# danieleschmidt/AV-Separation-Transformer

Hardware: NVIDIA B200
Metric: separated utterance-sec/sec (higher is better)
Workload: dtype bf16

## Files before the change

av-separation-transformer_b200/csrc/avsep_api.cu:

```cuda
#include "../../include/avsep.h"
#include "kernels.h"

#include <cuda_runtime.h>
#include <math.h>
#include <stdio.h>
#include <stdlib.h>
#include <string.h>

#include <functional>
#include <map>
#include <string>
#include <vector>

using namespace avsep;

namespace {

std::string g_create_error;

__global__ void op_to_f32_kernel(const __nv_bfloat16* in, float* out, size_t n) {
  size_t i = blockIdx.x * static_cast<size_t>(blockDim.x) + threadIdx.x;
  if (i < n) out[i] = __bfloat162float(in[i]);
}

__global__ void interp_rows_kernel(const float* __restrict__ x, float* __restrict__ out, int N, int T, int d,
                                   float scale) {
  const int t = blockIdx.x, b = blockIdx.y;
  const float sp = fmaxf(scale * (static_cast<float>(t) + 0.5f) - 0.5f, 0.0f);
  int i0 = static_cast<int>(sp);
  if (i0 > N - 1) i0 = N - 1;
  const int i1 = min(i0 + 1, N - 1);
  const float w1 = sp - static_cast<float>(i0), w0 = 1.0f - w1;
  const float* r0 = x + (static_cast<size_t>(b) * N + i0) * d;
  const float* r1 = x + (static_cast<size_t>(b) * N + i1) * d;
  float* o = out + (static_cast<size_t>(b) * T + t) * d;
  for (int c = threadIdx.x; c < d; c += blockDim.x) o[c] = w0 * r0[c] + w1 * r1[c];
}

__global__ void spin_kernel(unsigned long long ns) {
  unsigned long long t0, t;
  asm volatile("mov.u64 %0, %globaltimer;" : "=l"(t0));
  do {
    asm volatile("mov.u64 %0, %globaltimer;" : "=l"(t));
  } while (t - t0 < ns);
}

struct GraphKey {
  int B, T, N, Hh, Ww;
  const void *mixed, *frames, *sep, *masks, *ws;
  const int *lens, *frame_lens;
  bool operator==(const GraphKey& o) const {
    return B == o.B && T == o.T && N == o.N && Hh == o.Hh && Ww == o.Ww && mixed == o.mixed && frames == o.frames &&
           sep == o.sep && masks == o.masks && ws == o.ws && lens == o.lens && frame_lens == o.frame_lens;
  }
};
struct GraphEntry {
  GraphKey key;
  cudaGraphExec_t exec = nullptr;
  int64_t launches = 0;
  uint64_t last_use = 0;
};

struct HostTensor {
  std::vector<float> data;
  std::vector<int64_t> shape;
};

struct LayerW {
  const void *w_in, *wo, *w1, *w2;
  const float *b_in, *bo, *b1, *b2, *n1g, *n1b, *n2g, *n2b;
};

struct Workspace {
  int B = 0, T = 0, N = 0, Hh = 0, Ww = 0;
  const int *lens = nullptr, *frame_lens = nullptr;
  size_t bytes = 0;
  void *xp, *h1, *a_op, *qkv_a, *attn_a, *ffn_a;
  float *x_a, *y_a;
  void *pooled, *v_op, *qkv_v, *attn_v, *ffn_v;
  float *x_v, *y_v, *kvn;
  void* kvb;
};

}

struct avsep_handle {
  avsep_config cfg{};
  int Fp = 0;
  int num_sms = 148;
  std::string err;
  std::map<std::string, HostTensor> host_w;
  bool finalized = false;
  bool use_graph = true;
  int attn_tc = 1;
  bool two_stream = true;
  cudaStream_t aux_stream = nullptr;
  cudaEvent_t ev_fork = nullptr, ev_join = nullptr;
  std::vector<GraphEntry> graphs;
  uint64_t graph_clock = 0;
  cudaStream_t cap_stream = nullptr;
  int profile_spin_us = 3000;
  uint8_t* d_weights = nullptr;
  size_t weight_bytes = 0;
  const void *wc1 = nullptr, *wc2 = nullptr, *wproj = nullptr, *wkv_all = nullptr, *wdec0 = nullptr, *wdec3 = nullptr;
  const float *bc1 = nullptr, *bc2 = nullptr, *bproj = nullptr, *bkv_all = nullptr, *bdec0 = nullptr, *bdec3 = nullptr;
  const float *pe_a = nullptr, *pe_v = nullptr, *fng = nullptr, *fnb = nullptr;
  CnnWeights cnn{};
  const uint8_t *cnn_w2_slabs = nullptr, *cnn_w3_rows = nullptr;
  std::vector<LayerW> enc_a, enc_v, fus;
  const uint8_t *xs_a = nullptr, *xs_v = nullptr, *xs_f = nullptr;
  bool xs_f_decoder = false;
  const uint8_t *xs_a_np = nullptr, *xs_v_np = nullptr;
  bool xs_v_kvp = false;
  void* own_ws = nullptr;
  size_t own_ws_bytes = 0;
  struct HostSlot {
    float* io[4] = {nullptr, nullptr, nullptr, nullptr};
    size_t cap[4] = {0, 0, 0, 0};
    std::vector<cudaEvent_t> ev;
    cudaEvent_t ev_start = nullptr, ev_end = nullptr;
    cudaEvent_t ev_lane[3] = {nullptr, nullptr, nullptr};
  } slot[AVSEP_HOST_SLOTS];
  std::vector<void*> shared_owned, shared_mapped;
  float* synth_waves = nullptr;
  size_t synth_cap = 0;
  cudaStream_t hs[3] = {nullptr, nullptr, nullptr};
  int host_chunk = 0;
  bool pdl = true;
  int host_lanes = 0;
  void* host_ws = nullptr;
  size_t host_ws_bytes = 0;
  cudaStream_t host_comp[3] = {nullptr, nullptr, nullptr};
  bool debug = false;
  std::map<std::string, std::pair<float*, size_t>> snaps;
  int64_t launches = 0;
  bool profile = false;
  cudaStream_t prof_stream = nullptr;
  std::vector<cudaEvent_t> ev_pool;
  size_t ev_used = 0;
  std::vector<std::pair<const char*, size_t>> ev_marks;
  std::map<std::string, std::pair<int64_t, double>> prof;
};

namespace {

int fail(avsep_handle* h, const std::string& msg) {
  if (h) h->err = msg; else g_create_error = msg;
  return 1;
}

int prof_begin(avsep_handle* h, const char* label) {
  if (h->ev_used + 2 > h->ev_pool.size()) {
    for (int i = 0; i < 64; ++i) {
      cudaEvent_t e;
      if (cudaEventCreate(&e) != cudaSuccess) return 1;
      h->ev_pool.push_back(e);
    }
  }
  h->ev_marks.emplace_back(label, h->ev_used);
  cudaEventRecord(h->ev_pool[h->ev_used], h->prof_stream);
  return 0;
}
void prof_end(avsep_handle* h) {
  cudaEventRecord(h->ev_pool[h->ev_used + 1], h->prof_stream);
  h->ev_used += 2;
}

#define CKL(label, expr)                                                \
  do {                                                                  \
    if (h->profile && prof_begin(h, label)) return fail(h, "profiling: cudaEventCreate failed"); \
    const char* _e = (expr);                                            \
    if (_e != nullptr) return fail(h, std::string(_e) + " [" #expr "]"); \
    if (h->profile) prof_end(h);                                        \
    ++h->launches;                                                      \
  } while (0)
#define CK(expr) CKL("other", expr)

#define CUDA_OK(expr)                                                                           \
  do {                                                                                          \
    cudaError_t _c = (expr);                                                                    \
    if (_c != cudaSuccess) return fail(h, std::string(#expr ": ") + cudaGetErrorString(_c));    \
  } while (0)

size_t align_up(size_t v, size_t a) { return (v + a - 1) / a * a; }

void drop_graphs(avsep_handle* h) {
  for (auto& g : h->graphs)
    if (g.exec) cudaGraphExecDestroy(g.exec);
  h->graphs.clear();
}

size_t op_size(const avsep_handle* h) { return h->cfg.precision == AVSEP_PREC_TF32 ? 4 : 2; }

size_t carve_workspace(const avsep_handle* h, Workspace& w, uint8_t* base, int B, int T, int N, int Hh, int Ww) {
  const size_t d = h->cfg.d_model, os = op_size(h);
  const size_t Ma = static_cast<size_t>(B) * T, Map = static_cast<size_t>(B) * (T + 2), Mv = static_cast<size_t>(B) * N;
  size_t off = 0;
  auto take = [&](size_t bytes) {
    void* p = base ? base + off : nullptr;
    off += align_up(bytes, 1024);
    return p;
  };
  w.B = B; w.T = T; w.N = N; w.Hh = Hh; w.Ww = Ww;
  w.xp = take(Map * h->Fp * os);
  w.h1 = take(Map * d * os);
  w.x_a = static_cast<float*>(take(Ma * d * 4));
  w.y_a = static_cast<float*>(take(Ma * d * 4));
  w.a_op = take(Ma * d * os);
  w.qkv_a = take(Ma * 3 * d * os);
  w.attn_a = take(Ma * d * os);
  w.ffn_a = take(Ma * 4 * d * os);
  w.pooled = take(Mv * 128 * os);
  w.x_v = static_cast<float*>(take(Mv * d * 4));
  w.y_v = static_cast<float*>(take(Mv * d * 4));
  w.v_op = take(Mv * d * os);
  w.qkv_v = take(Mv * 3 * d * os);
  w.attn_v = take(Mv * d * os);
  w.ffn_v = take(Mv * 4 * d * os);
  w.kvn = static_cast<float*>(take(Mv * h->cfg.num_fusion_layers * 2 * d * 4));
  w.kvb = take(Ma * h->cfg.num_fusion_layers * 2 * d * os);
  w.bytes = off;
  return off;
}

int check_shape(avsep_handle* h, int B, int T, int N, int Hh, int Ww) {
  if (!h->finalized) return fail(h, "weights not finalized: call avsep_finalize_weights first");
  if (B < 1 || T < 1 || N < 1 || Hh < 1 || Ww < 1) return fail(h, "empty input: B, T, N, H, W must be >= 1");
  if (T > 5000 || N > 5000) return fail(h, "sequence longer than the positional table (max_len=5000, model.py:286)");
  if (B > 65535) return fail(h, "batch above 65535 utterances per call (grid dimension of the per-utterance kernels): split it");
  return 0;
}

int get_workspace(avsep_handle* h, Workspace& w, void* user_ws, size_t user_bytes, int B, int T, int N, int Hh, int Ww) {
  const size_t need = carve_workspace(h, w, nullptr, B, T, N, Hh, Ww);
  uint8_t* base = nullptr;
  if (user_ws != nullptr) {
    if (user_bytes < need) return fail(h, "workspace too small: see avsep_workspace_bytes");
    if ((reinterpret_cast<uintptr_t>(user_ws) & 1023) != 0) return fail(h, "workspace must be 1024-byte aligned");
    base = static_cast<uint8_t*>(user_ws);
  } else {
    if (h->own_ws_bytes < need) {
      drop_graphs(h);
      if (h->own_ws) cudaFree(h->own_ws);
      h->own_ws = nullptr;
      h->own_ws_bytes = 0;
      CUDA_OK(cudaMalloc(&h->own_ws, need));
      h->own_ws_bytes = need;
    }
    base = static_cast<uint8_t*>(h->own_ws);
  }
  carve_workspace(h, w, base, B, T, N, Hh, Ww);
  return 0;
}

int snapshot(avsep_handle* h, cudaStream_t s, const char* name, const void* ptr, size_t count, bool is_op) {
  if (!h->debug) return 0;
  auto& slot = h->snaps[name];
  if (slot.second < count) {
    if (slot.first) cudaFree(slot.first);
    slot.first = nullptr;
    CUDA_OK(cudaMalloc(&slot.first, count * sizeof(float)));
  }
  slot.second = count;
  if (is_op && h->cfg.precision == AVSEP_PREC_BF16) {
    op_to_f32_kernel<<<static_cast<unsigned>((count + 255) / 256), 256, 0, s>>>(
        static_cast<const __nv_bfloat16*>(ptr), slot.first, count);
  } else {
    CUDA_OK(cudaMemcpyAsync(slot.first, ptr, count * sizeof(float), cudaMemcpyDeviceToDevice, s));
  }
  return 0;
}

const char* run_visual_cnn(avsep_handle* h, cudaStream_t s, const float* frames, int M, int Hh, int Ww, void* pooled,
                           unsigned long long* trace = nullptr, const int* frame_lens = nullptr, int N = 1) {
  if (Hh == 32 && Ww == 32 && h->cfg.precision == AVSEP_PREC_BF16)
    return launch_visual_cnn_tc(s, frames, M, h->cnn, h->cnn_w2_slabs, h->cnn_w3_rows, pooled, h->num_sms, trace,
                                frame_lens, N);
  return launch_visual_cnn(s, h->cfg.precision, frames, M, Hh, Ww, h->cnn, pooled, h->num_sms, frame_lens, N);
}

GemmProblem dense(const void* A, int M, int K, const void* W, int N) {
  GemmProblem p{};
  p.A = A; p.lda = K; p.rowsA = M; p.M = M; p.W = W; p.ldw = K; p.N = N; p.K = K; p.taps = 1;
  return p;
}

int linear(avsep_handle* h, cudaStream_t s, const char* label, const void* A, int M, int K, const void* W,
           const float* bias, int N, int act, float* out_f32, void* out_op) {
  const GemmProblem p = dense(A, M, K, W, N);
  GemmEpilogue e;
  e.bias = bias; e.act = act;
  if (act == ACT_GELU && h->cfg.precision == AVSEP_PREC_BF16 && out_f32 == nullptr) e.act = ACT_GELU_BF16;
  e.out_f32 = out_f32; e.ld_f32 = N;
  e.out_op = out_op; e.ld_op = N;
  CKL(label, launch_gemm(s, h->cfg.precision, p, e, h->num_sms));
  return 0;
}

int gemm_resid_ln(avsep_handle* h, cudaStream_t s, const char* label, const GemmProblem& p, GemmEpilogue e,
                  const float* resid, float* x_out, const float* g, const float* b, void* out_op, int rows_out,
                  float* y) {
  const int prec = h->cfg.precision;
  if (gemm_ln_fusable(p.N)) {
    e.kind = EPI_LN;
    e.resid = resid;
    e.out_f32 = x_out; e.ld_f32 = p.N;
    e.ln_gamma = g; e.ln_beta = b;
    e.out_op = out_op; e.ld_op = p.N;
    CKL(label, launch_gemm(s, prec, p, e, h->num_sms));
    return 0;
  }
  e.kind = EPI_STD;
  e.out_op = nullptr;
  if (resid != nullptr) {
    e.out_f32 = y; e.ld_f32 = p.N;
    CKL(label, launch_gemm(s, prec, p, e, h->num_sms));
    CKL("add_layernorm", launch_add_layernorm(s, prec, resid, y, g, b, x_out, out_op, rows_out, p.N));
  } else {
    e.out_f32 = x_out; e.ld_f32 = p.N;
    CKL(label, launch_gemm(s, prec, p, e, h->num_sms));
    CKL("add_layernorm", launch_add_layernorm(s, prec, x_out, nullptr, g, b, nullptr, out_op, rows_out, p.N));
  }
  return 0;
}

int linear_resid_ln(avsep_handle* h, cudaStream_t s, const char* label, const void* A, int M, int K, const void* W,
                    const float* bias, int N, float* x, const float* g, const float* b, void* out_op, float* y) {
  GemmEpilogue e;
  e.bias = bias;
  return gemm_resid_ln(h, s, label, dense(A, M, K, W, N), e, x, x, g, b, out_op, M, y);
}

bool stack_fusable(const avsep_handle* h, int len) {
  return h->xs_a != nullptr && xformer_stack_usable(h->cfg.precision, h->cfg.d_model, h->cfg.nhead, len);
}

struct Plan {
  bool stack_a = false, stack_v = false;
  bool stack_f = false;
  bool pro = false;
  bool kvp = false;
  bool dec = false;
  bool fork = false;
};

Plan forward_plan(const avsep_handle* h, int T, int N) {
  Plan p;
  p.stack_a = stack_fusable(h, T);
  p.stack_v = stack_fusable(h, N);
  p.stack_f = p.stack_a && p.stack_v;
  p.pro = !h->debug;
  p.kvp = p.stack_f && h->xs_v_kvp && !h->debug &&
          xformer_kvp_usable(h->cfg.num_fusion_layers * 2 * h->cfg.d_model, N, T);
  p.dec = p.stack_f && h->xs_f_decoder && !h->debug;
  p.fork = h->two_stream && !h->profile && !h->debug;
  return p;
}

int run_stack(avsep_handle* h, cudaStream_t s, int which, StackProblem sp) {
  const bool pro = sp.pro_a != nullptr;
  sp.wstream = which == 0 ? (pro ? h->xs_a : h->xs_a_np) : which == 1 ? (pro ? h->xs_v : h->xs_v_np) : h->xs_f;
  sp.n_layers = which == 2 ? h->cfg.num_fusion_layers : h->cfg.num_encoder_layers;
  sp.cross = which == 2;
  if (sp.cross) sp.kv_ld = sp.n_layers * 2 * h->cfg.d_model;
  sp.act = sp.cross ? ACT_GELU : ACT_RELU;
  sp.F = h->cfg.freq_bins; sp.S = h->cfg.num_speakers;
  CKL(which == 0 ? "layer.audio_enc" : which == 1 ? "layer.visual_enc" : sp.masks ? "layer.fusion_decoder" : "layer.fusion",
      launch_xformer_stack(s, sp, h->num_sms));
  return 0;
}

constexpr int FFN_FUSED_MIN_ROWS = 2048;

int ffn_sublayer(avsep_handle* h, cudaStream_t s, const LayerW& w, int act, int M, float* x, void* a_op, void* ffn,
                 float* y, const float* g, const float* b) {
  const int d = h->cfg.d_model;
  if (ffn_fusable(h->cfg.precision, d) && M >= FFN_FUSED_MIN_ROWS) {
    CKL("ffn.fused", launch_ffn_fused(s, a_op, w.w1, w.b1, w.w2, w.b2, act, x, x, g, b, a_op, M, h->num_sms, nullptr));
    return 0;
  }
  if (linear(h, s, "gemm.ffn1", a_op, M, d, w.w1, w.b1, 4 * d, act, nullptr, ffn)) return 1;
  return linear_resid_ln(h, s, "gemm.ffn2", ffn, M, 4 * d, w.w2, w.b2, d, x, g, b, a_op, y);
}

int encoder_stack(avsep_handle* h, cudaStream_t s, const std::vector<LayerW>& layers, int B, int L, float* x,
                  float* y, void* a_op, void* qkv, void* attn, void* ffn, const float* final_g, const float* final_b,
                  const int* lens = nullptr) {
  const int d = h->cfg.d_model, H = h->cfg.nhead, M = B * L, prec = h->cfg.precision;
  const size_t os = op_size(h);
  for (size_t l = 0; l < layers.size(); ++l) {
    const LayerW& w = layers[l];
    if (linear(h, s, "gemm.qkv", a_op, M, d, w.w_in, w.b_in, 3 * d, ACT_NONE, nullptr, qkv)) return 1;
    AttnProblem ap{};
    ap.q = qkv; ap.ldq = 3 * d;
    ap.k = static_cast<const uint8_t*>(qkv) + static_cast<size_t>(d) * os;
    ap.v = static_cast<const uint8_t*>(qkv) + static_cast<size_t>(2 * d) * os;
    ap.ldkv = 3 * d;
    ap.out = attn; ap.ldo = d;
    ap.B = B; ap.H = H; ap.hd = d / H; ap.Lq = L; ap.Lk = L; ap.lerp_src = 0; ap.tc_mode = h->attn_tc;
    ap.k_lens = lens;
    CKL("attn.self", launch_attention(s, prec, ap));
    if (linear_resid_ln(h, s, "gemm.out_proj", attn, M, d, w.wo, w.bo, d, x, w.n2g, w.n2b, a_op, y)) return 1;
    const bool last = (l + 1 == layers.size());
    if (ffn_sublayer(h, s, w, ACT_RELU, M, x, a_op, ffn, y, last ? final_g : layers[l + 1].n1g,
                     last ? final_b : layers[l + 1].n1b))
      return 1;
  }
  return 0;
}

int audio_frontend(avsep_handle* h, cudaStream_t s, Workspace& w, const float* mixed, const Plan& pl) {
  h->prof_stream = s;
  const int d = h->cfg.d_model, F = h->cfg.freq_bins, B = w.B, T = w.T, prec = h->cfg.precision;
  const int Map = B * (T + 2);
  CKL("prep_audio", launch_prep_audio(s, prec, mixed, w.xp, B, F, T, h->Fp, w.lens));
  {
    GemmProblem p{};
    p.A = w.xp; p.lda = h->Fp; p.rowsA = Map; p.M = Map; p.W = h->wc1; p.ldw = 3 * h->Fp; p.N = d; p.K = h->Fp;
    p.taps = 3; p.tap_stride = h->Fp; p.row_shift = -1;
    GemmEpilogue e;
    e.bias = h->bc1; e.act = ACT_RELU; e.rowmap = ROW_PAD2PAD; e.Lp = T + 2;
    e.lens = w.lens;
    e.out_op = w.h1; e.ld_op = d;
    CKL("gemm.conv1d_0", launch_gemm(s, prec, p, e, h->num_sms));
  }
  if (pl.stack_a && pl.pro) return 0;
  {
    GemmProblem p{};
    p.A = w.h1; p.lda = d; p.rowsA = Map; p.M = Map; p.W = h->wc2; p.ldw = 3 * d; p.N = d; p.K = d;
    p.taps = 3; p.tap_stride = d; p.row_shift = -1;
    GemmEpilogue e;
    e.bias = h->bc2; e.act = ACT_RELU; e.rowmap = ROW_PAD2COMPACT; e.Lp = T + 2;
    e.pe = h->pe_a;
    if (pl.stack_a) {
      e.out_f32 = w.x_a; e.ld_f32 = d;
      CKL("gemm.conv1d_2", launch_gemm(s, prec, p, e, h->num_sms));
    } else if (gemm_resid_ln(h, s, "gemm.conv1d_2", p, e, nullptr, w.x_a, h->enc_a[0].n1g, h->enc_a[0].n1b, w.a_op,
                             B * T, w.y_a)) {
      return 1;
    }
  }
  return snapshot(h, s, "audio_embed", w.x_a, static_cast<size_t>(B) * T * d, false);
}

int visual_frontend(avsep_handle* h, cudaStream_t s, Workspace& w, const float* frames, const Plan& pl) {
  h->prof_stream = s;
  const int d = h->cfg.d_model, B = w.B, N = w.N;
  const int Mv = B * N;
  CKL("visual_cnn", run_visual_cnn(h, s, frames, Mv, w.Hh, w.Ww, w.pooled, nullptr, w.frame_lens, N));
  if (snapshot(h, s, "visual_pool", w.pooled, static_cast<size_t>(Mv) * 128, true)) return 1;
  if (pl.stack_v && pl.pro) return 0;
  const GemmProblem p = dense(w.pooled, Mv, 128, h->wproj, d);
  GemmEpilogue e;
  e.bias = h->bproj; e.pe = h->pe_v; e.pe_period = N;
  if (pl.stack_v) {
    e.out_f32 = w.x_v; e.ld_f32 = d;
    CKL("gemm.frame_proj", launch_gemm(s, h->cfg.precision, p, e, h->num_sms));
  } else if (gemm_resid_ln(h, s, "gemm.frame_proj", p, e, nullptr, w.x_v, h->enc_v[0].n1g, h->enc_v[0].n1b, w.v_op, Mv,
                           w.y_v)) {
    return 1;
  }
  return snapshot(h, s, "visual_embed", w.x_v, static_cast<size_t>(Mv) * d, false);
}

int fusion_stack_fused(avsep_handle* h, cudaStream_t s, Workspace& w, const Plan& pl, const float* mixed,
                       float* separated, float* masks) {
  h->prof_stream = s;
  const int d = h->cfg.d_model, B = w.B, T = w.T;
  const int Ma = B * T, Lf = h->cfg.num_fusion_layers;
  if (!pl.kvp) {
    CKL("lerp_kv", launch_lerp_rows(s, w.x_v, d, B, w.N, T, d, w.attn_a, d, w.frame_lens, w.lens));
    if (linear(h, s, "gemm.cross_kv", w.attn_a, Ma, d, h->wkv_all, h->bkv_all, Lf * 2 * d, ACT_NONE, nullptr, w.kvb)) return 1;
  }
  StackProblem sp{};
  sp.x_in = w.x_a; sp.fin_gamma = h->fng; sp.fin_beta = h->fnb; sp.kv = w.kvb;
  sp.B = B; sp.L = T; sp.lens = w.lens;
  if (pl.dec) {
    sp.mixed = mixed; sp.separated = separated; sp.masks = masks;
    return run_stack(h, s, 2, sp);
  }
  sp.out_x = h->debug ? w.x_a : nullptr; sp.out_op = w.a_op;
  if (run_stack(h, s, 2, sp)) return 1;
  return snapshot(h, s, "fused", w.a_op, static_cast<size_t>(Ma) * d, true);
}

int fusion_stack(avsep_handle* h, cudaStream_t s, Workspace& w, int L_src) {
  h->prof_stream = s;
  const int d = h->cfg.d_model, H = h->cfg.nhead, B = w.B, T = w.T, prec = h->cfg.precision;
  const int Ma = B * T, Mv = B * L_src, Lf = h->cfg.num_fusion_layers;
  if (linear(h, s, "gemm.cross_kv", w.v_op, Mv, d, h->wkv_all, h->bkv_all, Lf * 2 * d, ACT_NONE, w.kvn, nullptr)) return 1;
  for (int l = 0; l < Lf; ++l) {
    const LayerW& fw = h->fus[l];
    if (linear(h, s, "gemm.cross_q", w.a_op, Ma, d, fw.w_in, fw.b_in, d, ACT_NONE, nullptr, w.qkv_a)) return 1;
    AttnProblem ap{};
    ap.q = w.qkv_a; ap.ldq = d;
    ap.k = w.kvn + static_cast<size_t>(l) * 2 * d;
    ap.v = w.kvn + static_cast<size_t>(l) * 2 * d + d;
    ap.ldkv = Lf * 2 * d;
    ap.out = w.attn_a; ap.ldo = d;
    ap.B = B; ap.H = H; ap.hd = d / H; ap.Lq = T; ap.Lk = T; ap.lerp_src = L_src; ap.tc_mode = h->attn_tc;
    ap.k_lens = w.lens; ap.src_lens = w.frame_lens;
    {
      AttnProblem tp = ap;
      tp.lerp_src = 0;
      __nv_bfloat16* kvi = static_cast<__nv_bfloat16*>(w.qkv_a) + static_cast<size_t>(Ma) * d;
      tp.k = kvi; tp.v = kvi + d; tp.ldkv = 2 * d;
      if (attention_tc_wanted(prec, tp)) {
        CKL("lerp_kv", launch_lerp_rows(s, w.kvn + static_cast<size_t>(l) * 2 * d, Lf * 2 * d, B, L_src, T, 2 * d, kvi, 2 * d,
                                        w.frame_lens, w.lens));
        ap = tp;
      }
    }
    CKL("attn.cross", launch_attention(s, prec, ap));
    if (linear_resid_ln(h, s, "gemm.out_proj", w.attn_a, Ma, d, fw.wo, fw.bo, d, w.x_a, fw.n2g, fw.n2b, w.a_op, w.y_a))
      return 1;
    const bool last = (l + 1 == Lf);
    if (ffn_sublayer(h, s, fw, ACT_GELU, Ma, w.x_a, w.a_op, w.ffn_a, w.y_a, last ? h->fng : h->fus[l + 1].n1g,
                     last ? h->fnb : h->fus[l + 1].n1b))
      return 1;
  }
  return snapshot(h, s, "fused", w.a_op, static_cast<size_t>(Ma) * d, true);
}

int decoder_stage(avsep_handle* h, cudaStream_t s, Workspace& w, const float* mixed, float* separated, float* masks) {
  h->prof_stream = s;
  const int d = h->cfg.d_model, F = h->cfg.freq_bins, S = h->cfg.num_speakers, B = w.B, T = w.T;
  const int Ma = B * T;
  if (linear(h, s, "gemm.dec0", w.a_op, Ma, d, h->wdec0, h->bdec0, 2 * d, ACT_GELU, nullptr, w.ffn_a)) return 1;
  GemmEpilogue e;
  e.kind = EPI_TAIL;
  e.bias = h->bdec3;
  e.mixed = mixed; e.masks = masks; e.separated = separated; e.F = F; e.S = S; e.T = T;
  e.lens = w.lens;
  CKL("gemm.dec3_tail", launch_gemm(s, h->cfg.precision, dense(w.ffn_a, Ma, 2 * d, h->wdec3, S * F), e, h->num_sms));
  return 0;
}

int forward_device(avsep_handle* h, cudaStream_t s, Workspace& w, const float* mixed, const float* frames,
                   float* separated, float* masks) {
  const int d = h->cfg.d_model;
  const int Ma = w.B * w.T, Mv = w.B * w.N;
  const Plan pl = forward_plan(h, w.T, w.N);
  h->prof_stream = s;
  if (h->profile && h->profile_spin_us > 0) spin_kernel<<<1, 1, 0, s>>>(1000ull * h->profile_spin_us);
  cudaStream_t sv = s;
  if (pl.fork) {
    if (h->aux_stream == nullptr) {
      CUDA_OK(cudaStreamCreateWithFlags(&h->aux_stream, cudaStreamNonBlocking));
      CUDA_OK(cudaEventCreateWithFlags(&h->ev_fork, cudaEventDisableTiming));
      CUDA_OK(cudaEventCreateWithFlags(&h->ev_join, cudaEventDisableTiming));
    }
    sv = h->aux_stream;
    CUDA_OK(cudaEventRecord(h->ev_fork, s));
    CUDA_OK(cudaStreamWaitEvent(sv, h->ev_fork, 0));
  }
  if (visual_frontend(h, sv, w, frames, pl)) return 1;
  if (pl.stack_v) {
    StackProblem sp{};
    sp.x_in = w.x_v; sp.B = w.B; sp.L = w.N; sp.lens = w.frame_lens; sp.kvp_lens = w.lens;
    if (pl.pro) {
      sp.pro_a = w.pooled; sp.pro_taps = 1; sp.pro_k = 128; sp.pro_pitch = w.N; sp.pro_rows = Mv; sp.pe = h->pe_v;
    }
    if (pl.kvp) {
      sp.kvp_out = w.kvb; sp.kvp_L = w.T; sp.kvp_n = sp.kvp_ld = h->cfg.num_fusion_layers * 2 * d;
    } else {
      sp.out_x = w.x_v; sp.out_op = pl.stack_f ? nullptr : w.v_op;
    }
    if (run_stack(h, sv, 1, sp)) return 1;
  } else if (encoder_stack(h, sv, h->enc_v, w.B, w.N, w.x_v, w.y_v, w.v_op, w.qkv_v, w.attn_v, w.ffn_v, nullptr, nullptr,
                           w.frame_lens)) {
    return 1;
  }
  if (snapshot(h, sv, "visual_enc", w.x_v, static_cast<size_t>(Mv) * d, false)) return 1;
  if (audio_frontend(h, s, w, mixed, pl)) return 1;
  if (pl.stack_a) {
    StackProblem sp{};
    sp.x_in = w.x_a; sp.out_x = w.x_a; sp.out_op = pl.stack_f ? nullptr : w.a_op;
    sp.fin_gamma = h->fus[0].n1g; sp.fin_beta = h->fus[0].n1b;
    sp.B = w.B; sp.L = w.T; sp.lens = w.lens;
    if (pl.pro) {
      sp.pro_a = w.h1; sp.pro_relu = 1; sp.pro_taps = 3; sp.pro_k = d; sp.pro_pitch = w.T + 2;
      sp.pro_rows = w.B * (w.T + 2); sp.pe = h->pe_a;
    }
    if (run_stack(h, s, 0, sp)) return 1;
  } else if (encoder_stack(h, s, h->enc_a, w.B, w.T, w.x_a, w.y_a, w.a_op, w.qkv_a, w.attn_a, w.ffn_a, h->fus[0].n1g,
                           h->fus[0].n1b, w.lens)) {
    return 1;
  }
  if (snapshot(h, s, "audio_enc", w.x_a, static_cast<size_t>(Ma) * d, false)) return 1;
  if (pl.fork) {
    CUDA_OK(cudaEventRecord(h->ev_join, sv));
    CUDA_OK(cudaStreamWaitEvent(s, h->ev_join, 0));
  }
  if (pl.stack_f ? fusion_stack_fused(h, s, w, pl, mixed, separated, masks) : fusion_stack(h, s, w, w.N)) return 1;
  return pl.dec ? 0 : decoder_stage(h, s, w, mixed, separated, masks);
}

int forward_cached(avsep_handle* h, cudaStream_t s, Workspace& w, const void* ws_base, const float* mixed,
                   const float* frames, float* separated, float* masks) {
  if (!h->use_graph || h->profile || h->debug) return forward_device(h, s, w, mixed, frames, separated, masks);
  const GraphKey key{w.B, w.T, w.N, w.Hh, w.Ww, mixed, frames, separated, masks, ws_base, w.lens, w.frame_lens};
  GraphEntry* ent = nullptr;
  for (auto& g : h->graphs)
    if (g.key == key) { ent = &g; break; }
  if (ent == nullptr) {
    if (h->graphs.size() >= 64) {
      size_t victim = 0;
      for (size_t i = 1; i < h->graphs.size(); ++i)
        if (h->graphs[i].last_use < h->graphs[victim].last_use) victim = i;
      if (h->graphs[victim].exec) cudaGraphExecDestroy(h->graphs[victim].exec);
      h->graphs.erase(h->graphs.begin() + victim);
    }
    GraphEntry g;
    g.key = key;
    g.last_use = ++h->graph_clock;
    h->graphs.push_back(g);
    return forward_device(h, s, w, mixed, frames, separated, masks);
  }
  ent->last_use = ++h->graph_clock;
  if (ent->exec == nullptr) {
    if (h->cap_stream == nullptr) CUDA_OK(cudaStreamCreateWithFlags(&h->cap_stream, cudaStreamNonBlocking));
    CUDA_OK(cudaStreamBeginCapture(h->cap_stream, cudaStreamCaptureModeRelaxed));
    const int rc = forward_device(h, h->cap_stream, w, mixed, frames, separated, masks);
    cudaGraph_t graph = nullptr;
    const cudaError_t ce = cudaStreamEndCapture(h->cap_stream, &graph);
    if (rc != 0) {
      if (graph) cudaGraphDestroy(graph);
      return 1;
    }
    if (ce != cudaSuccess) return fail(h, std::string("cudaStreamEndCapture: ") + cudaGetErrorString(ce));
    const cudaError_t ci = cudaGraphInstantiate(&ent->exec, graph, 0);
    cudaGraphDestroy(graph);
    if (ci != cudaSuccess) {
      ent->exec = nullptr;
      return fail(h, std::string("cudaGraphInstantiate: ") + cudaGetErrorString(ci));
    }
    ent->launches = h->launches;
  }
  h->launches = ent->launches;
  CUDA_OK(cudaGraphLaunch(ent->exec, s));
  return 0;
}

const HostTensor* find_w(avsep_handle* h, const std::string& key, std::initializer_list<int64_t> shape) {
  auto it = h->host_w.find(key);
  if (it == h->host_w.end()) {
    h->err = "missing weight: " + key;
    return nullptr;
  }
  std::vector<int64_t> want(shape);
  if (it->second.shape != want) {
    h->err = "bad shape for weight: " + key;
    return nullptr;
  }
  return &it->second;
}

struct HostLayer {
  const HostTensor *w_in, *b_in, *wo, *bo, *w1, *b1, *w2, *b2, *n1g, *n1b, *n2g, *n2b;
};
bool find_layer(avsep_handle* h, const std::string& p, bool cross, int64_t d, HostLayer& t) {
  const std::string at = p + (cross ? ".cross_attn." : ".self_attn."), f1 = p + (cross ? ".ff.0." : ".linear1."),
                    f2 = p + (cross ? ".ff.3." : ".linear2.");
  return (t.w_in = find_w(h, at + "in_proj_weight", {3 * d, d})) && (t.b_in = find_w(h, at + "in_proj_bias", {3 * d})) &&
         (t.wo = find_w(h, at + "out_proj.weight", {d, d})) && (t.bo = find_w(h, at + "out_proj.bias", {d})) &&
         (t.w1 = find_w(h, f1 + "weight", {4 * d, d})) && (t.b1 = find_w(h, f1 + "bias", {4 * d})) &&
         (t.w2 = find_w(h, f2 + "weight", {d, 4 * d})) && (t.b2 = find_w(h, f2 + "bias", {d})) &&
         (t.n1g = find_w(h, p + ".norm1.weight", {d})) && (t.n1b = find_w(h, p + ".norm1.bias", {d})) &&
         (t.n2g = find_w(h, p + ".norm2.weight", {d})) && (t.n2b = find_w(h, p + ".norm2.bias", {d}));
}

struct ArenaBuilder {
  std::vector<uint8_t> bytes;
  std::vector<std::function<void(const uint8_t*)>> fills;
  template <typename T>
  void add(const T*& field, const void* src, size_t n) {
    const size_t off = align_up(bytes.size(), 256);
    bytes.resize(off + n);
    memcpy(bytes.data() + off, src, n);
    fills.push_back([&field, off](const uint8_t* base) { field = reinterpret_cast<const T*>(base + off); });
  }
  void add_f32(const float*& field, const float* src, size_t n) { add(field, src, n * 4); }
  void add_f32(const float*& field, const HostTensor* t) { add_f32(field, t->data.data(), t->data.size()); }
  void add_op(const void*& field, const float* src, size_t n, bool tf32) {
    if (tf32) {
      std::vector<float> tmp(n);
      for (size_t i = 0; i < n; ++i) {
        uint32_t u;
        memcpy(&u, &src[i], 4);
        if ((u & 0x7f800000u) != 0x7f800000u) u = (u + 0x1000u) & 0xffffe000u;
        memcpy(&tmp[i], &u, 4);
      }
      return add(field, tmp.data(), n * 4);
    }
    std::vector<uint16_t> tmp(n);
    for (size_t i = 0; i < n; ++i) tmp[i] = f2bf(src[i]);
    add(field, tmp.data(), n * 2);
  }
  void add_op(const void*& field, const HostTensor* t, bool tf32) { add_op(field, t->data.data(), t->data.size(), tf32); }
  void patch(const uint8_t* base) {
    for (auto& f : fills) f(base);
  }
};

void add_layer(ArenaBuilder& ar, LayerW& w, const HostLayer& t, bool cross, int64_t d, bool tf32) {
  ar.add_op(w.w_in, t.w_in->data.data(), static_cast<size_t>(cross ? d : 3 * d) * d, tf32);
  if (cross) ar.add_f32(w.b_in, t.b_in->data.data(), d);
  ar.add_op(w.wo, t.wo, tf32);
  ar.add_op(w.w1, t.w1, tf32);
  ar.add_op(w.w2, t.w2, tf32);
  if (!cross) ar.add_f32(w.b_in, t.b_in);
  ar.add_f32(w.bo, t.bo);
  ar.add_f32(w.b1, t.b1);
  ar.add_f32(w.b2, t.b2);
  ar.add_f32(w.n1g, t.n1g);
  ar.add_f32(w.n1b, t.n1b);
  ar.add_f32(w.n2g, t.n2g);
  ar.add_f32(w.n2b, t.n2b);
}

void pack_stream_layer(const HostLayer& t, bool cross, int d, const float* b0, std::vector<float>& vecs, uint8_t* dst) {
  xformer_pack_vecs(t.b_in->data.data(), cross ? d : 3 * d, t.bo->data.data(), t.b1->data.data(), t.b2->data.data(),
                    t.n1g->data.data(), t.n1b->data.data(), t.n2g->data.data(), t.n2b->data.data(), vecs.data(), b0);
  (cross ? xformer_pack_cross : xformer_pack_self)(t.w_in->data.data(), t.wo->data.data(), t.w1->data.data(),
                                                   t.w2->data.data(), vecs.data(), dst);
}

}

extern "C" {

int avsep_create(const avsep_config* cfg, avsep_handle** out) {
  if (!cfg || !out) return fail(nullptr, "avsep_create: null argument");
  *out = nullptr;
  if (cfg->freq_bins < 1 || cfg->d_model < 8 || cfg->nhead < 1 || cfg->num_encoder_layers < 1 ||
      cfg->num_fusion_layers < 1 || cfg->num_speakers < 1)
    return fail(nullptr, "avsep_create: all sizes must be positive (at least one encoder and one fusion layer)");
  if (cfg->d_model % cfg->nhead != 0) return fail(nullptr, "avsep_create: d_model must be divisible by nhead");
  const int hd = cfg->d_model / cfg->nhead;
  if (hd != 16 && hd != 32 && hd != 64 && hd != 128)
    return fail(nullptr, "avsep_create: head dim (d_model/nhead) must be 16, 32, 64 or 128");
  if (cfg->d_model % 8 != 0 || cfg->d_model > 1024)
    return fail(nullptr, "avsep_create: d_model must be a multiple of 8 and <= 1024");
  if (cfg->precision != AVSEP_PREC_BF16 && cfg->precision != AVSEP_PREC_TF32)
    return fail(nullptr, "avsep_create: unknown precision");
  int ndev = 0;
  if (cudaGetDeviceCount(&ndev) != cudaSuccess || ndev <= 0)
    return fail(nullptr, "avsep_create: no CUDA device (this library has no CPU path)");
  if (cfg->device < 0 || cfg->device >= ndev) return fail(nullptr, "avsep_create: bad device ordinal");
  cudaDeviceProp prop;
  if (cudaGetDeviceProperties(&prop, cfg->device) != cudaSuccess) return fail(nullptr, "avsep_create: device query failed");
  if (prop.major != 10) return fail(nullptr, "avsep_create: kernels are built for sm_100a (B200) only");
  if (cudaSetDevice(cfg->device) != cudaSuccess) return fail(nullptr, "avsep_create: cudaSetDevice failed");
  if (const char* e = tma_init()) return fail(nullptr, e);
  if (const char* e = fft512_init_tables()) return fail(nullptr, e);
  avsep_handle* h = new avsep_handle();
  h->cfg = *cfg;
  h->Fp = (cfg->freq_bins + 7) / 8 * 8;
  h->num_sms = prop.multiProcessorCount;
  *out = h;
  if (const char* e = getenv("AVSEP_OPTS")) {
    std::string opts(e);
    size_t pos = 0;
    while (pos < opts.size()) {
      size_t end = opts.find(',', pos);
      if (end == std::string::npos) end = opts.size();
      const std::string kv = opts.substr(pos, end - pos);
      const size_t eq = kv.find('=');
      if (eq != std::string::npos && avsep_set_option(h, kv.substr(0, eq).c_str(), atoi(kv.c_str() + eq + 1)) != 0)
        fprintf(stderr, "avsep: AVSEP_OPTS: option '%s' not accepted\n", kv.c_str());
      pos = end + 1;
    }
  }
  return 0;
}

void avsep_destroy(avsep_handle* h) {
  if (!h) return;
  cudaSetDevice(h->cfg.device);
  if (h->d_weights) cudaFree(h->d_weights);
  if (h->own_ws) cudaFree(h->own_ws);
  for (auto& sl : h->slot) {
    for (float* ptr : sl.io)
      if (ptr) cudaFree(ptr);
    for (cudaEvent_t e : sl.ev) cudaEventDestroy(e);
    if (sl.ev_start) cudaEventDestroy(sl.ev_start);
    if (sl.ev_end) cudaEventDestroy(sl.ev_end);
    for (cudaEvent_t e : sl.ev_lane)
      if (e) cudaEventDestroy(e);
  }
  for (void* ptr : h->shared_mapped) cudaIpcCloseMemHandle(ptr);
  for (void* ptr : h->shared_owned) cudaFree(ptr);
  if (h->synth_waves) cudaFree(h->synth_waves);
  if (h->host_ws) cudaFree(h->host_ws);
  for (auto& kv : h->snaps)
    if (kv.second.first) cudaFree(kv.second.first);
  for (cudaEvent_t e : h->ev_pool) cudaEventDestroy(e);
  for (auto& g : h->graphs)
    if (g.exec) cudaGraphExecDestroy(g.exec);
  if (h->cap_stream) cudaStreamDestroy(h->cap_stream);
  if (h->aux_stream) cudaStreamDestroy(h->aux_stream);
  if (h->ev_fork) cudaEventDestroy(h->ev_fork);
  if (h->ev_join) cudaEventDestroy(h->ev_join);
  for (int i = 0; i < 3; ++i) {
    if (h->hs[i]) cudaStreamDestroy(h->hs[i]);
    if (h->host_comp[i]) cudaStreamDestroy(h->host_comp[i]);
  }
  delete h;
}

const char* avsep_last_error(const avsep_handle* h) { return h ? h->err.c_str() : g_create_error.c_str(); }

int avsep_set_weight(avsep_handle* h, const char* key, const void* host_data, int32_t dtype, const int64_t* shape,
                     int32_t ndim) {
  if (!h || !key || (!host_data && ndim >= 0) || ndim < 0 || ndim > 8) return fail(h, "avsep_set_weight: bad argument");
  if (dtype == AVSEP_DTYPE_I64) return 0;
  if (dtype != AVSEP_DTYPE_F32) return fail(h, "avsep_set_weight: only fp32 tensors are accepted");
  HostTensor t;
  size_t n = 1;
  for (int i = 0; i < ndim; ++i) {
    if (shape[i] < 0) return fail(h, "avsep_set_weight: negative dimension");
    t.shape.push_back(shape[i]);
    n *= static_cast<size_t>(shape[i]);
  }
  t.data.assign(static_cast<const float*>(host_data), static_cast<const float*>(host_data) + n);
  h->host_w[key] = std::move(t);
  h->finalized = false;
  return 0;
}

int avsep_finalize_weights(avsep_handle* h, void* cuda_stream) {
  if (!h) return 1;
  cudaStream_t s = static_cast<cudaStream_t>(cuda_stream);
  CUDA_OK(cudaSetDevice(h->cfg.device));
  const int64_t d = h->cfg.d_model, F = h->cfg.freq_bins, S = h->cfg.num_speakers, Fp = h->Fp;
  const int Le = h->cfg.num_encoder_layers, Lf = h->cfg.num_fusion_layers;
  const bool tf32 = h->cfg.precision == AVSEP_PREC_TF32;
#define GETW(var, key, ...)                                  \
  const HostTensor* var = find_w(h, key, {__VA_ARGS__});     \
  if (!var) return 1;
  GETW(c0w, "audio_encoder.input_proj.0.weight", d, F, 3);
  GETW(c0b, "audio_encoder.input_proj.0.bias", d);
  GETW(c2w, "audio_encoder.input_proj.2.weight", d, d, 3);
  GETW(c2b, "audio_encoder.input_proj.2.bias", d);
  GETW(pea, "audio_encoder.pos_enc.pe", 1, 5000, d);
  GETW(pev, "visual_encoder.pos_enc.pe", 1, 5000, d);
  GETW(projw, "visual_encoder.frame_proj.weight", d, 128);
  GETW(projb, "visual_encoder.frame_proj.bias", d);
  GETW(fng, "fusion.norm.weight", d);
  GETW(fnb, "fusion.norm.bias", d);
  GETW(dec0w, "decoder.decoder.0.weight", 2 * d, d);
  GETW(dec0b, "decoder.decoder.0.bias", 2 * d);
  GETW(dec3w, "decoder.decoder.3.weight", S * F, 2 * d);
  GETW(dec3b, "decoder.decoder.3.bias", S * F);
  std::vector<HostLayer> enc[2] = {std::vector<HostLayer>(Le), std::vector<HostLayer>(Le)}, fus(Lf);
  for (int l = 0; l < Le; ++l)
    if (!find_layer(h, "audio_encoder.transformer.layers." + std::to_string(l), false, d, enc[0][l]) ||
        !find_layer(h, "visual_encoder.transformer.layers." + std::to_string(l), false, d, enc[1][l]))
      return 1;
  for (int l = 0; l < Lf; ++l)
    if (!find_layer(h, "fusion.layers." + std::to_string(l), true, d, fus[l])) return 1;
  const int cins[3] = {1, 32, 64}, couts[3] = {32, 64, 128}, idx[3] = {0, 3, 6};
  std::vector<float> folded[3], fbias[3];
  for (int c = 0; c < 3; ++c) {
    const std::string cp = "visual_encoder.conv." + std::to_string(idx[c]);
    const std::string bp = "visual_encoder.conv." + std::to_string(idx[c] + 1);
    GETW(w, cp + ".weight", couts[c], cins[c], 3, 3);
    GETW(b, cp + ".bias", couts[c]);
    GETW(g, bp + ".weight", couts[c]);
    GETW(be, bp + ".bias", couts[c]);
    GETW(mu, bp + ".running_mean", couts[c]);
    GETW(var, bp + ".running_var", couts[c]);
    const int K = 9 * cins[c];
    folded[c].assign(static_cast<size_t>(couts[c]) * K, 0.f);
    fbias[c].assign(couts[c], 0.f);
    for (int o = 0; o < couts[c]; ++o) {
      const float scale = g->data[o] / sqrtf(var->data[o] + 1e-5f);
      fbias[c][o] = (b->data[o] - mu->data[o]) * scale + be->data[o];
      for (int ci = 0; ci < cins[c]; ++ci)
        for (int tap = 0; tap < 9; ++tap)
          folded[c][static_cast<size_t>(o) * K + tap * cins[c] + ci] =
              w->data[(static_cast<size_t>(o) * cins[c] + ci) * 9 + tap] * scale;
    }
  }
#undef GETW
  const int n_kv = static_cast<int>(Lf * 2 * d);
  std::vector<float> wkv(static_cast<size_t>(n_kv) * d), bkv(n_kv);
  for (int l = 0; l < Lf; ++l) {
    memcpy(wkv.data() + static_cast<size_t>(l) * 2 * d * d, fus[l].w_in->data.data() + d * d, sizeof(float) * 2 * d * d);
    memcpy(bkv.data() + static_cast<size_t>(l) * 2 * d, fus[l].b_in->data.data() + d, sizeof(float) * 2 * d);
  }

  ArenaBuilder ar;
  h->enc_a.assign(Le, LayerW{});
  h->enc_v.assign(Le, LayerW{});
  h->fus.assign(Lf, LayerW{});
  {
    std::vector<float> p0(static_cast<size_t>(d) * 3 * Fp, 0.f), p2(static_cast<size_t>(d) * 3 * d, 0.f);
    for (int64_t o = 0; o < d; ++o)
      for (int64_t c = 0; c < F; ++c)
        for (int tap = 0; tap < 3; ++tap) p0[(o * 3 + tap) * Fp + c] = c0w->data[(o * F + c) * 3 + tap];
    for (int64_t o = 0; o < d; ++o)
      for (int64_t c = 0; c < d; ++c)
        for (int tap = 0; tap < 3; ++tap) p2[(o * 3 + tap) * d + c] = c2w->data[(o * d + c) * 3 + tap];
    ar.add_op(h->wc1, p0.data(), p0.size(), tf32);
    ar.add_op(h->wc2, p2.data(), p2.size(), tf32);
  }
  ar.add_f32(h->bc1, c0b);
  ar.add_f32(h->bc2, c2b);
  ar.add_f32(h->pe_a, pea);
  ar.add_f32(h->pe_v, pev);
  for (int l = 0; l < Le; ++l) add_layer(ar, h->enc_a[l], enc[0][l], false, d, tf32);
  for (int l = 0; l < Le; ++l) add_layer(ar, h->enc_v[l], enc[1][l], false, d, tf32);
  {
    std::vector<uint32_t> p1(visual_cnn_pack_sizes(1)), p2(visual_cnn_pack_sizes(2)), p3(visual_cnn_pack_sizes(3));
    visual_cnn_pack(folded[0].data(), folded[1].data(), folded[2].data(), p1.data(), p2.data(), p3.data());
    std::vector<uint8_t> tc2(visual_cnn_tc_w2_bytes()), tc3(visual_cnn_tc_w3_bytes());
    visual_cnn_tc_pack(folded[1].data(), folded[2].data(), tc2.data(), tc3.data());
    ar.add(h->cnn_w2_slabs, tc2.data(), tc2.size());
    ar.add(h->cnn_w3_rows, tc3.data(), tc3.size());
    ar.add(h->cnn.w1, p1.data(), p1.size() * 4);
    ar.add(h->cnn.w2, p2.data(), p2.size() * 4);
    ar.add(h->cnn.w3, p3.data(), p3.size() * 4);
    visual_cnn_pack(folded[0].data(), folded[1].data(), folded[2].data(), p1.data(), p2.data(), p3.data(), true);
    ar.add(h->cnn.w1l, p1.data(), p1.size() * 4);
    ar.add(h->cnn.w2l, p2.data(), p2.size() * 4);
    ar.add(h->cnn.w3l, p3.data(), p3.size() * 4);
    ar.add_f32(h->cnn.b1, fbias[0].data(), 32);
    ar.add_f32(h->cnn.b2, fbias[1].data(), 64);
    ar.add_f32(h->cnn.b3, fbias[2].data(), 128);
  }
  ar.add_op(h->wproj, projw, tf32);
  ar.add_f32(h->bproj, projb);
  for (int l = 0; l < Lf; ++l) add_layer(ar, h->fus[l], fus[l], true, d, tf32);
  ar.add_op(h->wkv_all, wkv.data(), wkv.size(), tf32);
  ar.add_f32(h->bkv_all, bkv.data(), bkv.size());
  ar.add_f32(h->fng, fng);
  ar.add_f32(h->fnb, fnb);
  ar.add_op(h->wdec0, dec0w, tf32);
  ar.add_op(h->wdec3, dec3w, tf32);
  ar.add_f32(h->bdec0, dec0b);
  ar.add_f32(h->bdec3, dec3b);

  h->xs_a = h->xs_v = h->xs_f = nullptr;
  if (xformer_stack_usable(h->cfg.precision, static_cast<int>(d), h->cfg.nhead, 1)) {
    const size_t sb = xformer_stream_bytes(false), cb = xformer_stream_bytes(true);
    const size_t pro_a = xformer_pro_bytes(3, static_cast<int>(d)), pro_v = xformer_pro_bytes(1, 128);
    h->xs_v_kvp = xformer_kvp_usable(n_kv, 1, 1);
    h->xs_f_decoder = xformer_decoder_usable(static_cast<int>(S), static_cast<int>(F));
    std::vector<uint8_t> xa(pro_a + Le * sb), xv(pro_v + Le * sb + (h->xs_v_kvp ? xformer_kvp_bytes(n_kv) : 0)),
        xf(Lf * cb + (h->xs_f_decoder ? xformer_decoder_bytes(static_cast<int>(S), static_cast<int>(F)) : 0));
    std::vector<float> vecs(xformer_vec_floats());
    xformer_pack_pro(c2w->data.data(), static_cast<int>(3 * d), 3, 3, static_cast<int>(d), xa.data());
    xformer_pack_pro(projw->data.data(), 128, 1, 1, 128, xv.data());
    for (int l = 0; l < Le; ++l) {
      pack_stream_layer(enc[0][l], false, d, l == 0 ? c2b->data.data() : nullptr, vecs, xa.data() + pro_a + l * sb);
      pack_stream_layer(enc[1][l], false, d, l == 0 ? projb->data.data() : nullptr, vecs, xv.data() + pro_v + l * sb);
    }
    if (h->xs_v_kvp) xformer_pack_kvp(wkv.data(), bkv.data(), n_kv, xv.data() + pro_v + Le * sb);
    for (int l = 0; l < Lf; ++l) pack_stream_layer(fus[l], true, d, nullptr, vecs, xf.data() + l * cb);
    if (h->xs_f_decoder)
      xformer_pack_decoder(dec0w->data.data(), dec0b->data.data(), dec3w->data.data(), dec3b->data.data(),
                           static_cast<int>(S), static_cast<int>(F), xf.data() + Lf * cb);
    ar.add(h->xs_a, xa.data(), xa.size());
    ar.add(h->xs_v, xv.data(), xv.size());
    ar.add(h->xs_f, xf.data(), xf.size());
  }
  drop_graphs(h);
  if (h->d_weights) cudaFree(h->d_weights);
  h->d_weights = nullptr;
  CUDA_OK(cudaMalloc(&h->d_weights, ar.bytes.size()));
  h->weight_bytes = ar.bytes.size();
  CUDA_OK(cudaMemcpyAsync(h->d_weights, ar.bytes.data(), ar.bytes.size(), cudaMemcpyHostToDevice, s));
  CUDA_OK(cudaStreamSynchronize(s));
  ar.patch(h->d_weights);
  if (h->xs_a != nullptr) {
    h->xs_a_np = h->xs_a + xformer_pro_bytes(3, h->cfg.d_model);
    h->xs_v_np = h->xs_v + xformer_pro_bytes(1, 128);
  }
  h->finalized = true;
  return 0;
}

size_t avsep_workspace_bytes(avsep_handle* h, int32_t B, int32_t T, int32_t N, int32_t Hh, int32_t Ww) {
  if (!h || B < 1 || T < 1 || N < 1) return 0;
  Workspace w;
  return carve_workspace(h, w, nullptr, B, T, N, Hh, Ww);
}

int avsep_forward(avsep_handle* h, const float* mixed_spec, const float* lip_frames, int32_t B, int32_t T, int32_t N,
                  int32_t Hh, int32_t Ww, float* separated, float* masks, void* workspace, size_t workspace_bytes,
                  void* cuda_stream) {
  return avsep_forward_varlen(h, mixed_spec, lip_frames, nullptr, nullptr, B, T, N, Hh, Ww, separated, masks, workspace,
                              workspace_bytes, cuda_stream);
}

int avsep_forward_varlen(avsep_handle* h, const float* mixed_spec, const float* lip_frames, const int32_t* lengths,
                         const int32_t* frame_lengths, int32_t B, int32_t T, int32_t N, int32_t Hh, int32_t Ww,
                         float* separated, float* masks, void* workspace, size_t workspace_bytes, void* cuda_stream) {
  if (!h) return 1;
  if (!mixed_spec || !lip_frames || !separated || !masks) return fail(h, "avsep_forward: null buffer");
  if (check_shape(h, B, T, N, Hh, Ww)) return 1;
  CUDA_OK(cudaSetDevice(h->cfg.device));
  Workspace w;
  if (get_workspace(h, w, workspace, workspace_bytes, B, T, N, Hh, Ww)) return 1;
  w.lens = lengths; w.frame_lens = frame_lengths;
  h->launches = 0;
  return forward_cached(h, static_cast<cudaStream_t>(cuda_stream), w, workspace ? workspace : h->own_ws, mixed_spec,
                        lip_frames, separated, masks);
}

namespace {
int host_submit(avsep_handle* h, const float* mixed_spec, const float* lip_frames, int B, int T, int N, int Hh, int Ww,
                float* separated, float* masks, int slot_id, cudaStream_t s, bool streaming) {
  if (!mixed_spec || !lip_frames || !separated || !masks) return fail(h, "avsep_forward_host: null buffer");
  if (slot_id < 0 || slot_id >= AVSEP_HOST_SLOTS) return fail(h, "avsep_forward_host_async: slot must be 0 .. AVSEP_HOST_SLOTS - 1");
  if (check_shape(h, B, T, N, Hh, Ww)) return 1;
  CUDA_OK(cudaSetDevice(h->cfg.device));
  avsep_handle::HostSlot& sl = h->slot[slot_id];
  const size_t F = h->cfg.freq_bins, S = h->cfg.num_speakers;
  const size_t mixed_per = F * T, frames_per = static_cast<size_t>(N) * Hh * Ww, out_per = S * F * T;
  const size_t need[4] = {B * mixed_per, B * frames_per, B * out_per, B * out_per};
  for (int i = 0; i < 4; ++i) {
    if (sl.cap[i] < need[i]) {
      if (sl.ev_end) CUDA_OK(cudaEventSynchronize(sl.ev_end));
      if (sl.io[i]) cudaFree(sl.io[i]);
      sl.io[i] = nullptr;
      sl.cap[i] = 0;
      CUDA_OK(cudaMalloc(&sl.io[i], need[i] * sizeof(float)));
      sl.cap[i] = need[i];
    }
  }
  float *io_mixed = sl.io[0], *io_frames = sl.io[1], *io_sep = sl.io[2], *io_masks = sl.io[3];
  if (h->hs[0] == nullptr) {
    for (int i = 0; i < 3; ++i) CUDA_OK(cudaStreamCreateWithFlags(&h->hs[i], cudaStreamNonBlocking));
  }
  auto make_event = [&](cudaEvent_t& e) -> int {
    if (e == nullptr) CUDA_OK(cudaEventCreateWithFlags(&e, cudaEventDisableTiming));
    return 0;
  };
  if (make_event(sl.ev_start) || make_event(sl.ev_end)) return 1;
  const int auto_chunk = streaming ? 128 : 56;
  const int want_chunk = h->host_chunk > 0 ? h->host_chunk : auto_chunk;
  const int Bc = want_chunk < B ? want_chunk : B;
  std::vector<int> starts, sizes;
  for (int b0 = 0; b0 < B; b0 += Bc) {
    starts.push_back(b0);
    sizes.push_back((B - b0) < Bc ? (B - b0) : Bc);
  }
  const int nchunks = static_cast<int>(starts.size());
  while (static_cast<int>(sl.ev.size()) < 2 * nchunks) {
    cudaEvent_t e;
    CUDA_OK(cudaEventCreateWithFlags(&e, cudaEventDisableTiming));
    sl.ev.push_back(e);
  }
  const int want_lanes = h->host_lanes > 0 ? h->host_lanes : (streaming ? 1 : 2);
  const int lanes = want_lanes > 3 ? 3 : want_lanes;
  Workspace wl[3];
  const size_t per_lane = carve_workspace(h, wl[0], nullptr, Bc, T, N, Hh, Ww);
  if (h->host_ws_bytes < per_lane * lanes) {
    CUDA_OK(cudaDeviceSynchronize());
    drop_graphs(h);
    if (h->host_ws) cudaFree(h->host_ws);
    h->host_ws = nullptr;
    h->host_ws_bytes = 0;
    CUDA_OK(cudaMalloc(&h->host_ws, per_lane * lanes));
    h->host_ws_bytes = per_lane * lanes;
  }
  for (int l = 0; l < lanes; ++l) {
    carve_workspace(h, wl[l], static_cast<uint8_t*>(h->host_ws) + l * per_lane, Bc, T, N, Hh, Ww);
    if (h->host_comp[l] == nullptr) CUDA_OK(cudaStreamCreateWithFlags(&h->host_comp[l], cudaStreamNonBlocking));
    if (make_event(sl.ev_lane[l])) return 1;
  }
  cudaStream_t s_in = h->hs[0], s_out = h->hs[2];
  CUDA_OK(cudaEventRecord(sl.ev_start, s));
  CUDA_OK(cudaStreamWaitEvent(s_in, sl.ev_start, 0));
  for (int l = 0; l < 3; ++l)
    if (sl.ev_lane[l]) CUDA_OK(cudaStreamWaitEvent(s_in, sl.ev_lane[l], 0));
  for (int l = 0; l < lanes; ++l) {
    CUDA_OK(cudaStreamWaitEvent(h->host_comp[l], sl.ev_start, 0));
    CUDA_OK(cudaStreamWaitEvent(h->host_comp[l], sl.ev_end, 0));
  }
  CUDA_OK(cudaStreamWaitEvent(s_out, sl.ev_start, 0));
  int64_t launches = 0;
  for (int c = 0; c < nchunks; ++c) {
    const size_t b0 = starts[c];
    const int bc = sizes[c];
    const int lane = c % lanes;
    cudaStream_t s_comp = h->host_comp[lane];
    CUDA_OK(cudaMemcpyAsync(io_mixed + b0 * mixed_per, mixed_spec + b0 * mixed_per, bc * mixed_per * 4,
                            cudaMemcpyHostToDevice, s_in));
    CUDA_OK(cudaMemcpyAsync(io_frames + b0 * frames_per, lip_frames + b0 * frames_per, bc * frames_per * 4,
                            cudaMemcpyHostToDevice, s_in));
    CUDA_OK(cudaEventRecord(sl.ev[2 * c], s_in));
    CUDA_OK(cudaStreamWaitEvent(s_comp, sl.ev[2 * c], 0));
    Workspace wc = wl[lane];
    wc.B = bc;
    if (forward_cached(h, s_comp, wc, static_cast<uint8_t*>(h->host_ws) + lane * per_lane, io_mixed + b0 * mixed_per,
                       io_frames + b0 * frames_per, io_sep + b0 * out_per, io_masks + b0 * out_per))
      return 1;
    launches += h->launches;
    CUDA_OK(cudaEventRecord(sl.ev[2 * c + 1], s_comp));
    CUDA_OK(cudaStreamWaitEvent(s_out, sl.ev[2 * c + 1], 0));
    CUDA_OK(cudaMemcpyAsync(separated + b0 * out_per, io_sep + b0 * out_per, bc * out_per * 4,
                            cudaMemcpyDeviceToHost, s_out));
    CUDA_OK(cudaMemcpyAsync(masks + b0 * out_per, io_masks + b0 * out_per, bc * out_per * 4,
                            cudaMemcpyDeviceToHost, s_out));
  }
  h->launches = launches;
  for (int l = 0; l < lanes; ++l) CUDA_OK(cudaEventRecord(sl.ev_lane[l], h->host_comp[l]));
  CUDA_OK(cudaEventRecord(sl.ev_end, s_out));
  return 0;
}
}

int avsep_forward_host(avsep_handle* h, const float* mixed_spec, const float* lip_frames, int32_t B, int32_t T,
                       int32_t N, int32_t Hh, int32_t Ww, float* separated, float* masks, void* cuda_stream) {
  if (!h) return 1;
  if (host_submit(h, mixed_spec, lip_frames, B, T, N, Hh, Ww, separated, masks, 0, static_cast<cudaStream_t>(cuda_stream), false))
    return 1;
  CUDA_OK(cudaEventSynchronize(h->slot[0].ev_end));
  return 0;
}

int avsep_forward_host_async(avsep_handle* h, const float* mixed_spec, const float* lip_frames, int32_t B, int32_t T,
                             int32_t N, int32_t Hh, int32_t Ww, float* separated, float* masks, int32_t slot,
                             void* cuda_stream) {
  if (!h) return 1;
  return host_submit(h, mixed_spec, lip_frames, B, T, N, Hh, Ww, separated, masks, slot,
                     static_cast<cudaStream_t>(cuda_stream), true);
}

int avsep_host_wait(avsep_handle* h, int32_t slot) {
  if (!h) return 1;
  if (slot < 0 || slot >= AVSEP_HOST_SLOTS) return fail(h, "avsep_host_wait: slot must be 0 .. AVSEP_HOST_SLOTS - 1");
  if (h->slot[slot].ev_end == nullptr) return 0;
  CUDA_OK(cudaSetDevice(h->cfg.device));
  CUDA_OK(cudaEventSynchronize(h->slot[slot].ev_end));
  return 0;
}

int avsep_synth_batch(avsep_handle* h, const avsep_synth_config* cfg, int32_t B, const double* amps, const double* freqs,
                      const double* phases, const float* noise, float* mixed_spec, float* lip_frames,
                      float* clean_specs, void* cuda_stream) {
  if (!h) return 1;
  if (!cfg || !amps || !freqs || !phases || !mixed_spec || !lip_frames) return fail(h, "avsep_synth_batch: null argument");
  if (B < 1) return fail(h, "avsep_synth_batch: empty batch");
  CUDA_OK(cudaSetDevice(h->cfg.device));
  SynthProblem p{};
  p.B = B; p.S = cfg->num_speakers; p.n = cfg->num_samples_audio; p.nfft = cfg->n_fft; p.hop = cfg->hop_length;
  p.nf = cfg->num_frames; p.Hh = cfg->frame_h; p.Ww = cfg->frame_w; p.duration = cfg->duration;
  p.amps = amps; p.freqs = freqs; p.phases = phases; p.noise = noise;
  p.mixed_spec = mixed_spec; p.lip_frames = lip_frames; p.clean_specs = clean_specs;
  if (p.S < 1 || p.n < 1) return fail(h, "avsep_synth_batch: bad geometry");
  const size_t need = static_cast<size_t>(B) * (p.S + 1) * p.n;
  if (h->synth_cap < need) {
    if (h->synth_waves) cudaFree(h->synth_waves);
    h->synth_waves = nullptr; h->synth_cap = 0;
    CUDA_OK(cudaMalloc(&h->synth_waves, need * sizeof(float)));
    h->synth_cap = need;
  }
  p.waves = h->synth_waves;
  h->launches = 0;
  CK(launch_synth(static_cast<cudaStream_t>(cuda_stream), p));
  h->launches = 3;
  return 0;
}

int avsep_eval_snr(avsep_handle* h, const float* separated, const float* targets, const float* mixed, int32_t B,
                   int32_t S, int32_t F, int32_t T, double* input_snr, double* output_snr, int32_t* best_perm,
                   double* si_snr, void* cuda_stream) {
  if (!h) return 1;
  if (!separated || !targets) return fail(h, "avsep_eval_snr: null argument");
  if (B < 1 || F < 1 || T < 1) return fail(h, "avsep_eval_snr: empty problem");
  CUDA_OK(cudaSetDevice(h->cfg.device));
  CK(launch_eval_snr(static_cast<cudaStream_t>(cuda_stream), separated, targets, mixed, B, S, F * T, input_snr,
                     output_snr, best_perm, si_snr));
  h->launches = 1;
  return 0;
}

int avsep_stft(avsep_handle* h, const float* waves, int32_t B, int32_t L, int32_t n_fft, int32_t hop_length,
               float* spec, float* mag, void* cuda_stream) {
  return avsep_stft_varlen(h, waves, nullptr, B, L, n_fft, hop_length, spec, mag, nullptr, cuda_stream);
}

int avsep_stft_varlen(avsep_handle* h, const float* waves, const int32_t* lengths, int32_t B, int32_t L, int32_t n_fft,
                      int32_t hop_length, float* spec, float* mag, int32_t* frame_lengths_out, void* cuda_stream) {
  if (!h) return 1;
  if (!waves || !spec) return fail(h, "avsep_stft: null argument");
  CUDA_OK(cudaSetDevice(h->cfg.device));
  CK(launch_stft_complex(static_cast<cudaStream_t>(cuda_stream), waves, lengths, B, L, n_fft, hop_length, spec, mag,
                         frame_lengths_out));
  h->launches = 1;
  return 0;
}

int avsep_istft(avsep_handle* h, const float* spec, const float* masks, int32_t B, int32_t S, int32_t T,
                int32_t n_fft, int32_t hop_length, int32_t L, float* waves, void* cuda_stream) {
  return avsep_istft_varlen(h, spec, masks, nullptr, B, S, T, n_fft, hop_length, L, waves, cuda_stream);
}

int avsep_istft_varlen(avsep_handle* h, const float* spec, const float* masks, const int32_t* lengths, int32_t B,
                       int32_t S, int32_t T, int32_t n_fft, int32_t hop_length, int32_t L, float* waves,
                       void* cuda_stream) {
  if (!h) return 1;
  if (!spec || !waves) return fail(h, "avsep_istft: null argument");
  CUDA_OK(cudaSetDevice(h->cfg.device));
  CK(launch_istft_masked(static_cast<cudaStream_t>(cuda_stream), spec, masks, lengths, B, S, T, n_fft, hop_length, L,
                         waves));
  h->launches = 1;
  return 0;
}

int64_t avsep_last_launch_count(const avsep_handle* h) { return h ? h->launches : 0; }

int avsep_shared_alloc(avsep_handle* h, size_t bytes, void** dev_ptr, unsigned char handle_out[AVSEP_IPC_HANDLE_BYTES]) {
  if (!h) return 1;
  if (!dev_ptr || !handle_out || bytes == 0) return fail(h, "avsep_shared_alloc: bad argument");
  static_assert(sizeof(cudaIpcMemHandle_t) == AVSEP_IPC_HANDLE_BYTES, "IPC handle size");
  CUDA_OK(cudaSetDevice(h->cfg.device));
  void* ptr = nullptr;
  CUDA_OK(cudaMalloc(&ptr, bytes));
  cudaIpcMemHandle_t ih;
  const cudaError_t ce = cudaIpcGetMemHandle(&ih, ptr);
  if (ce != cudaSuccess) {
    cudaFree(ptr);
    return fail(h, std::string("cudaIpcGetMemHandle: ") + cudaGetErrorString(ce));
  }
  memcpy(handle_out, &ih, sizeof ih);
  h->shared_owned.push_back(ptr);
  *dev_ptr = ptr;
  return 0;
}

int avsep_shared_free(avsep_handle* h, void* dev_ptr) {
  if (!h) return 1;
  for (size_t i = 0; i < h->shared_owned.size(); ++i)
    if (h->shared_owned[i] == dev_ptr) {
      CUDA_OK(cudaSetDevice(h->cfg.device));
      h->shared_owned.erase(h->shared_owned.begin() + i);
      CUDA_OK(cudaFree(dev_ptr));
      return 0;
    }
  return fail(h, "avsep_shared_free: pointer was not allocated by avsep_shared_alloc on this handle");
}

int avsep_shared_open(avsep_handle* h, const unsigned char handle[AVSEP_IPC_HANDLE_BYTES], void** dev_ptr) {
  if (!h) return 1;
  if (!handle || !dev_ptr) return fail(h, "avsep_shared_open: bad argument");
  CUDA_OK(cudaSetDevice(h->cfg.device));
  cudaIpcMemHandle_t ih;
  memcpy(&ih, handle, sizeof ih);
  void* ptr = nullptr;
  CUDA_OK(cudaIpcOpenMemHandle(&ptr, ih, cudaIpcMemLazyEnablePeerAccess));
  h->shared_mapped.push_back(ptr);
  *dev_ptr = ptr;
  return 0;
}

int avsep_shared_close(avsep_handle* h, void* dev_ptr) {
  if (!h) return 1;
  for (size_t i = 0; i < h->shared_mapped.size(); ++i)
    if (h->shared_mapped[i] == dev_ptr) {
      CUDA_OK(cudaSetDevice(h->cfg.device));
      h->shared_mapped.erase(h->shared_mapped.begin() + i);
      CUDA_OK(cudaIpcCloseMemHandle(dev_ptr));
      return 0;
    }
  return fail(h, "avsep_shared_close: pointer was not mapped by avsep_shared_open on this handle");
}

int avsep_copy_async(avsep_handle* h, void* dst, const void* src, size_t bytes, void* cuda_stream) {
  if (!h) return 1;
  if (!dst || !src) return fail(h, "avsep_copy_async: null buffer");
  if (bytes == 0) return 0;
  CUDA_OK(cudaSetDevice(h->cfg.device));
  CUDA_OK(cudaMemcpyAsync(dst, src, bytes, cudaMemcpyDefault, static_cast<cudaStream_t>(cuda_stream)));
  return 0;
}

int avsep_separate(avsep_handle* h, const float* masks, const float* mixed_spec, int32_t B, int32_t T, float* separated,
                   void* cuda_stream) {
  if (!h) return 1;
  if (!masks || !mixed_spec || !separated) return fail(h, "avsep_separate: null buffer");
  if (B < 1 || T < 1) return fail(h, "avsep_separate: B and T must be >= 1");
  CUDA_OK(cudaSetDevice(h->cfg.device));
  const char* e = launch_separate(static_cast<cudaStream_t>(cuda_stream), masks, mixed_spec, separated, B,
                                  h->cfg.num_speakers, h->cfg.freq_bins, T);
  return e ? fail(h, e) : 0;
}

namespace {
int make_flag_set(avsep_handle* h, uint32_t* const* flags, int32_t n, FlagSet& f, const char* who) {
  if (!flags || n < 1 || n > FlagSet::MAX) return fail(h, std::string(who) + ": 1 .. 16 flags");
  f.n = n;
  for (int i = 0; i < n; ++i) {
    if (!flags[i] || (reinterpret_cast<uintptr_t>(flags[i]) & 3)) return fail(h, std::string(who) + ": bad flag pointer");
    f.ptr[i] = flags[i];
  }
  return 0;
}
}

int avsep_flag_signal(avsep_handle* h, uint32_t* const* flags, int32_t n, uint32_t value, void* cuda_stream) {
  if (!h) return 1;
  FlagSet f;
  if (make_flag_set(h, flags, n, f, "avsep_flag_signal")) return 1;
  CUDA_OK(cudaSetDevice(h->cfg.device));
  const char* e = launch_flag_signal(static_cast<cudaStream_t>(cuda_stream), f, value);
  return e ? fail(h, e) : 0;
}

int avsep_flag_wait(avsep_handle* h, uint32_t* const* flags, int32_t n, uint32_t value, double timeout_s,
                    void* cuda_stream) {
  if (!h) return 1;
  FlagSet f;
  if (make_flag_set(h, flags, n, f, "avsep_flag_wait")) return 1;
  if (!(timeout_s > 0.0) || timeout_s > 3600.0) return fail(h, "avsep_flag_wait: timeout_s must be in (0, 3600]");
  CUDA_OK(cudaSetDevice(h->cfg.device));
  const char* e = launch_flag_wait(static_cast<cudaStream_t>(cuda_stream), f, value, timeout_s);
  return e ? fail(h, e) : 0;
}

int avsep_audio_encoder(avsep_handle* h, const float* mixed_spec, int32_t B, int32_t T, float* out_BTd,
                        void* cuda_stream) {
  if (!h) return 1;
  if (!mixed_spec || !out_BTd) return fail(h, "avsep_audio_encoder: null buffer");
  if (check_shape(h, B, T, 1, 1, 1)) return 1;
  CUDA_OK(cudaSetDevice(h->cfg.device));
  cudaStream_t s = static_cast<cudaStream_t>(cuda_stream);
  Workspace w;
  if (get_workspace(h, w, nullptr, 0, B, T, 1, 1, 1)) return 1;
  const int d = h->cfg.d_model, Ma = B * T;
  h->launches = 0;
  if (audio_frontend(h, s, w, mixed_spec, Plan{})) return 1;
  if (encoder_stack(h, s, h->enc_a, B, T, w.x_a, w.y_a, w.a_op, w.qkv_a, w.attn_a, w.ffn_a, nullptr, nullptr)) return 1;
  CUDA_OK(cudaMemcpyAsync(out_BTd, w.x_a, static_cast<size_t>(Ma) * d * 4, cudaMemcpyDeviceToDevice, s));
  return 0;
}

int avsep_visual_encoder(avsep_handle* h, const float* lip_frames, int32_t B, int32_t N, int32_t Hh, int32_t Ww,
                         int32_t target_len, float* out_BTd, void* cuda_stream) {
  if (!h) return 1;
  if (!lip_frames || !out_BTd) return fail(h, "avsep_visual_encoder: null buffer");
  if (check_shape(h, B, 1, N, Hh, Ww)) return 1;
  if (target_len < 1) return fail(h, "avsep_visual_encoder: target_len must be >= 1");
  CUDA_OK(cudaSetDevice(h->cfg.device));
  cudaStream_t s = static_cast<cudaStream_t>(cuda_stream);
  Workspace w;
  if (get_workspace(h, w, nullptr, 0, B, 1, N, Hh, Ww)) return 1;
  const int d = h->cfg.d_model;
  h->launches = 0;
  if (visual_frontend(h, s, w, lip_frames, Plan{})) return 1;
  if (encoder_stack(h, s, h->enc_v, B, N, w.x_v, w.y_v, w.v_op, w.qkv_v, w.attn_v, w.ffn_v, nullptr, nullptr)) return 1;
  interp_rows_kernel<<<dim3(target_len, B), 128, 0, s>>>(w.x_v, out_BTd, N, target_len, d,
                                                         static_cast<float>(N) / static_cast<float>(target_len));
  CUDA_OK(cudaGetLastError());
  ++h->launches;
  return 0;
}

int avsep_fusion(avsep_handle* h, const float* audio_BTd, const float* visual_BLd, int32_t B, int32_t T, int32_t L,
                 float* out_BTd, void* cuda_stream) {
  if (!h) return 1;
  if (!audio_BTd || !visual_BLd || !out_BTd) return fail(h, "avsep_fusion: null buffer");
  if (check_shape(h, B, T, L, 1, 1)) return 1;
  if (L != T) return fail(h, "avsep_fusion: audio and visual must have the same length (model.py:131-133)");
  CUDA_OK(cudaSetDevice(h->cfg.device));
  cudaStream_t s = static_cast<cudaStream_t>(cuda_stream);
  Workspace w;
  if (get_workspace(h, w, nullptr, 0, B, T, L, 1, 1)) return 1;
  const int d = h->cfg.d_model, Ma = B * T, Mv = B * L, prec = h->cfg.precision;
  h->launches = 0;
  CUDA_OK(cudaMemcpyAsync(w.x_a, audio_BTd, static_cast<size_t>(Ma) * d * 4, cudaMemcpyDeviceToDevice, s));
  CKL("add_layernorm", launch_add_layernorm(s, prec, w.x_a, nullptr, h->fus[0].n1g, h->fus[0].n1b, nullptr, w.a_op, Ma, d));
  CKL("add_layernorm", launch_add_layernorm(s, prec, visual_BLd, nullptr, nullptr, nullptr, nullptr, w.v_op, Mv, d));
  const bool dbg = h->debug;
  h->debug = false;
  const int rc = fusion_stack(h, s, w, L);
  h->debug = dbg;
  if (rc) return 1;
  CKL("add_layernorm", launch_add_layernorm(s, PREC_TF32, w.x_a, nullptr, h->fng, h->fnb, nullptr, out_BTd, Ma, d));
  return 0;
}

int avsep_decoder(avsep_handle* h, const float* fused_BTd, const float* mixed_spec, int32_t B, int32_t T,
                  float* separated, float* masks, void* cuda_stream) {
  if (!h) return 1;
  if (!fused_BTd || !mixed_spec || !separated || !masks) return fail(h, "avsep_decoder: null buffer");
  if (check_shape(h, B, T, 1, 1, 1)) return 1;
  CUDA_OK(cudaSetDevice(h->cfg.device));
  cudaStream_t s = static_cast<cudaStream_t>(cuda_stream);
  Workspace w;
  if (get_workspace(h, w, nullptr, 0, B, T, 1, 1, 1)) return 1;
  const int d = h->cfg.d_model, Ma = B * T;
  h->launches = 0;
  CKL("add_layernorm", launch_add_layernorm(s, h->cfg.precision, fused_BTd, nullptr, nullptr, nullptr, nullptr, w.a_op, Ma, d));
  return decoder_stage(h, s, w, mixed_spec, separated, masks);
}

int avsep_set_debug(avsep_handle* h, int32_t enable) {
  if (!h) return 1;
  h->debug = enable != 0;
  return 0;
}

int avsep_debug_get_stage(avsep_handle* h, const char* name, float* host_out, size_t capacity, size_t* count) {
  if (!h || !name || !count) return fail(h, "avsep_debug_get_stage: bad argument");
  auto it = h->snaps.find(name);
  if (it == h->snaps.end()) return fail(h, std::string("no snapshot named ") + name);
  *count = it->second.second;
  if (host_out == nullptr) return 0;
  if (capacity < it->second.second) return fail(h, "avsep_debug_get_stage: buffer too small");
  CUDA_OK(cudaDeviceSynchronize());
  CUDA_OK(cudaMemcpy(host_out, it->second.first, it->second.second * sizeof(float), cudaMemcpyDeviceToHost));
  return 0;
}

int avsep_set_profile(avsep_handle* h, int32_t enable) {
  if (!h) return 1;
  h->profile = enable != 0;
  pdl_set(h->pdl && !h->profile);
  return 0;
}

int avsep_profile_report(avsep_handle* h, char* buf, size_t capacity, int32_t reset) {
  if (!h || !buf || capacity == 0) return fail(h, "avsep_profile_report: bad argument");
  CUDA_OK(cudaDeviceSynchronize());
  for (auto& mk : h->ev_marks) {
    float ms = 0.f;
    if (cudaEventElapsedTime(&ms, h->ev_pool[mk.second], h->ev_pool[mk.second + 1]) == cudaSuccess) {
      auto& slot = h->prof[mk.first];
      slot.first += 1;
      slot.second += ms;
    }
  }
  h->ev_marks.clear();
  h->ev_used = 0;
  std::string out;
  for (auto& kv : h->prof) {
    char line[160];
    snprintf(line, sizeof line, "%s %lld %.6f\n", kv.first.c_str(), static_cast<long long>(kv.second.first), kv.second.second);
    out += line;
  }
  if (out.size() + 1 > capacity) return fail(h, "avsep_profile_report: buffer too small");
  memcpy(buf, out.c_str(), out.size() + 1);
  if (reset) h->prof.clear();
  return 0;
}

int avsep_test_gemm(avsep_handle* h, const void* A, const void* W, const float* bias, float* out, int32_t M, int32_t N,
                    int32_t K, int32_t act, int32_t force_bn, void* cuda_stream) {
  if (!h) return 1;
  const GemmProblem p = dense(A, M, K, W, N);
  GemmEpilogue e;
  e.bias = bias; e.act = act; e.out_f32 = out; e.ld_f32 = N;
  CK(launch_gemm(static_cast<cudaStream_t>(cuda_stream), h->cfg.precision, p, e, h->num_sms, force_bn));
  return 0;
}

int avsep_test_gemm_ln(avsep_handle* h, const void* A, const void* W, const float* bias, float* x, const float* gamma,
                       const float* beta, void* out_op, int32_t M, int32_t N, int32_t K, void* cuda_stream) {
  if (!h) return 1;
  const GemmProblem p = dense(A, M, K, W, N);
  GemmEpilogue e;
  e.kind = EPI_LN;
  e.bias = bias; e.resid = x; e.out_f32 = x; e.ld_f32 = N; e.ln_gamma = gamma; e.ln_beta = beta;
  e.out_op = out_op; e.ld_op = N;
  CK(launch_gemm(static_cast<cudaStream_t>(cuda_stream), h->cfg.precision, p, e, h->num_sms));
  return 0;
}

int avsep_test_gemm_trace(avsep_handle* h, const void* A, const void* W, const float* bias, float* x_or_out,
                          const float* gamma, const float* beta, void* out_op, int32_t M, int32_t N, int32_t K,
                          int32_t ln, int32_t act, unsigned long long* trace_dev, void* cuda_stream) {
  if (!h) return 1;
  const GemmProblem p = dense(A, M, K, W, N);
  GemmEpilogue e;
  e.bias = bias; e.act = act;
  if (ln == 7) {
    e.kind = EPI_TAIL; e.act = ACT_NONE;
    e.S = 2; e.F = N / 2; e.T = act;
    e.mixed = gamma; e.masks = x_or_out; e.separated = static_cast<float*>(out_op);
  } else if (ln) {
    e.kind = EPI_LN;
    e.resid = x_or_out; e.out_f32 = x_or_out; e.ld_f32 = N; e.ln_gamma = gamma; e.ln_beta = beta;
    e.out_op = out_op; e.ld_op = N;
    if (ln == 2) e.resid = nullptr;
    if (ln == 3) e.out_f32 = nullptr;
    if (ln == 4) e.out_op = nullptr;
    if (ln == 5) { e.resid = nullptr; e.out_f32 = nullptr; }
    if (ln == 6) { e.ln_gamma = nullptr; }
  } else {
    e.out_op = out_op; e.ld_op = N;
    e.out_f32 = out_op ? nullptr : x_or_out; e.ld_f32 = N;
  }
  CK(launch_gemm(static_cast<cudaStream_t>(cuda_stream), h->cfg.precision, p, e, h->num_sms, 0, trace_dev));
  return 0;
}

int avsep_test_ffn_fused(avsep_handle* h, const void* a, const void* w1, const float* b1, const void* w2,
                         const float* b2, int32_t act, float* x_inout, const float* gamma, const float* beta,
                         void* out_op, int32_t M, void* cuda_stream) {
  if (!h) return 1;
  CK(launch_ffn_fused(static_cast<cudaStream_t>(cuda_stream), a, w1, b1, w2, b2, act,
                                                             x_inout, x_inout, gamma, beta, out_op, M, h->num_sms, nullptr));
  return 0;
}

int avsep_test_ffn_fused_trace(avsep_handle* h, const void* a, const void* w1, const float* b1, const void* w2,
                               const float* b2, int32_t act, float* x_inout, const float* gamma, const float* beta,
                               void* out_op, int32_t M, unsigned long long* trace_dev, void* cuda_stream) {
  if (!h) return 1;
  CK(launch_ffn_fused(static_cast<cudaStream_t>(cuda_stream), a, w1, b1, w2, b2, act,
                                                             x_inout, x_inout, gamma, beta, out_op, M, h->num_sms, trace_dev));
  return 0;
}

int avsep_test_xformer_stack(avsep_handle* h, int32_t which, const float* x_in, const void* kv, int32_t B, int32_t L,
                             float* out_x, void* out_op, int32_t final_ln, long long* trace_dev, void* cuda_stream) {
  if (!h) return 1;
  if (!h->finalized) return fail(h, "weights not finalized");
  if (which < 0 || which > 2) return fail(h, "test_xformer_stack: which must be 0, 1 or 2");
  if (h->xs_a == nullptr || !xformer_stack_usable(h->cfg.precision, h->cfg.d_model, h->cfg.nhead, L))
    return fail(h, "test_xformer_stack: the fused stack kernel does not support this configuration");
  StackProblem sp{};
  sp.x_in = x_in; sp.out_x = out_x; sp.out_op = out_op; sp.kv = kv; sp.B = B; sp.L = L; sp.trace = trace_dev;
  if (final_ln && which == 0) { sp.fin_gamma = h->fus[0].n1g; sp.fin_beta = h->fus[0].n1b; }
  if (final_ln && which == 2) { sp.fin_gamma = h->fng; sp.fin_beta = h->fnb; }
  h->prof_stream = static_cast<cudaStream_t>(cuda_stream);
  return run_stack(h, static_cast<cudaStream_t>(cuda_stream), which, sp);
}

int avsep_test_fusion_decoder(avsep_handle* h, const float* x_in, const void* kv, int32_t B, int32_t L, const float* mixed,
                              float* separated, float* masks, long long* trace_dev, void* cuda_stream) {
  if (!h) return 1;
  if (!h->finalized) return fail(h, "weights not finalized");
  if (h->xs_f == nullptr || !h->xs_f_decoder || !xformer_stack_usable(h->cfg.precision, h->cfg.d_model, h->cfg.nhead, L))
    return fail(h, "test_fusion_decoder: the fused stack kernel does not support this configuration");
  if (!mixed || !separated || !masks) return fail(h, "test_fusion_decoder: null buffer");
  StackProblem sp{};
  sp.x_in = x_in; sp.fin_gamma = h->fng; sp.fin_beta = h->fnb; sp.kv = kv; sp.B = B; sp.L = L; sp.trace = trace_dev;
  sp.mixed = mixed; sp.separated = separated; sp.masks = masks;
  h->prof_stream = static_cast<cudaStream_t>(cuda_stream);
  return run_stack(h, static_cast<cudaStream_t>(cuda_stream), 2, sp);
}

int avsep_set_option(avsep_handle* h, const char* name, int32_t value) {
  if (!h || !name) return 1;
  if (strcmp(name, "host_chunk") == 0) { h->host_chunk = value; return 0; }
  if (strcmp(name, "host_lanes") == 0) { h->host_lanes = value; return 0; }
  if (strcmp(name, "pdl") == 0) { h->pdl = value != 0; pdl_set(h->pdl && !h->profile); drop_graphs(h); return 0; }
  if (strcmp(name, "use_graph") == 0) { h->use_graph = value != 0; return 0; }
  if (strcmp(name, "two_stream") == 0) { h->two_stream = value != 0; drop_graphs(h); return 0; }
  if (strcmp(name, "attn_tc") == 0) { h->attn_tc = value; drop_graphs(h); return 0; }
  if (strcmp(name, "profile_spin_us") == 0) { h->profile_spin_us = value; return 0; }
  return fail(h, std::string("unknown option ") + name);
}

int avsep_test_conv1d(avsep_handle* h, const void* A_padded, const void* W3, const float* bias, float* out, int32_t B,
                      int32_t L, int32_t N, int32_t K, void* cuda_stream) {
  if (!h) return 1;
  GemmProblem p{};
  const int Mp = B * (L + 2);
  p.A = A_padded; p.lda = K; p.rowsA = Mp; p.M = Mp; p.W = W3; p.ldw = 3 * K; p.N = N; p.K = K;
  p.taps = 3; p.tap_stride = K; p.row_shift = -1;
  GemmEpilogue e;
  e.bias = bias; e.rowmap = ROW_PAD2COMPACT; e.Lp = L + 2; e.out_f32 = out; e.ld_f32 = N;
  CK(launch_gemm(static_cast<cudaStream_t>(cuda_stream), h->cfg.precision, p, e, h->num_sms));
  return 0;
}

int avsep_test_attention(avsep_handle* h, const void* q, const void* k, const void* v, void* out, int32_t B, int32_t H,
                         int32_t hd, int32_t Lq, int32_t Lk, int32_t lerp_src, void* cuda_stream) {
  if (!h) return 1;
  AttnProblem ap{};
  ap.q = q; ap.ldq = H * hd; ap.k = k; ap.v = v; ap.ldkv = H * hd; ap.out = out; ap.ldo = H * hd;
  ap.B = B; ap.H = H; ap.hd = hd; ap.Lq = Lq; ap.Lk = Lk; ap.lerp_src = lerp_src; ap.tc_mode = h->attn_tc;
  cudaStream_t s = static_cast<cudaStream_t>(cuda_stream);
  void* scratch = nullptr;
  if (lerp_src > 0) {
    AttnProblem tp = ap;
    tp.lerp_src = 0; tp.ldkv = 2 * H * hd;
    if (attention_tc_wanted(h->cfg.precision, tp)) {
      const int dm = H * hd;
      if (cudaMalloc(&scratch, static_cast<size_t>(B) * Lk * 2 * dm * 2) != cudaSuccess) return fail(h, "test_attention: cudaMalloc failed");
      tp.k = scratch; tp.v = static_cast<__nv_bfloat16*>(scratch) + dm;
      CK(launch_lerp_rows(s, static_cast<const float*>(k), dm, B, lerp_src, Lk, dm, scratch, 2 * dm));
      CK(launch_lerp_rows(s, static_cast<const float*>(v), dm, B, lerp_src, Lk, dm, static_cast<__nv_bfloat16*>(scratch) + dm, 2 * dm));
      ap = tp;
    }
  }
  const char* err = launch_attention(s, h->cfg.precision, ap);
  if (scratch) { cudaStreamSynchronize(s); cudaFree(scratch); }
  if (err) return fail(h, err);
  return 0;
}

int avsep_test_add_layernorm(avsep_handle* h, const float* x, const float* y, const float* gamma, const float* beta,
                             float* x_out, void* out_op, int32_t M, int32_t d, void* cuda_stream) {
  if (!h) return 1;
  CKL("add_layernorm", launch_add_layernorm(static_cast<cudaStream_t>(cuda_stream), h->cfg.precision, x, y, gamma, beta, x_out, out_op, M, d));
  return 0;
}

int avsep_test_visual_cnn(avsep_handle* h, const float* frames, int32_t M, int32_t Hh, int32_t Ww, void* pooled,
                          void* cuda_stream) {
  if (!h) return 1;
  if (!h->finalized) return fail(h, "weights not finalized");
  CK(run_visual_cnn(h, static_cast<cudaStream_t>(cuda_stream), frames, M, Hh, Ww, pooled));
  return 0;
}

int avsep_test_visual_cnn_trace(avsep_handle* h, const float* frames, int32_t M, void* pooled,
                                unsigned long long* trace_dev, void* cuda_stream) {
  if (!h) return 1;
  if (!h->finalized) return fail(h, "weights not finalized");
  CK(run_visual_cnn(h, static_cast<cudaStream_t>(cuda_stream), frames, M, 32, 32, pooled, trace_dev));
  return 0;
}

}
```

av-separation-transformer_b200/csrc/common.cuh:

```cuda
#pragma once

#include <cuda_runtime.h>
#include <cuda_bf16.h>
#include <cuda.h>
#include <stdint.h>
#include <stdio.h>

#ifndef AVSEP_WATCHDOG_CYCLES
#define AVSEP_WATCHDOG_CYCLES (4000000000ll)
#endif

namespace avsep {

__device__ __forceinline__ uint32_t smem_u32(const void* p) {
  return static_cast<uint32_t>(__cvta_generic_to_shared(p));
}

__device__ __forceinline__ float warp_sum(float v) {
#pragma unroll
  for (int o = 16; o > 0; o >>= 1) v += __shfl_xor_sync(0xffffffffu, v, o);
  return v;
}

__device__ __forceinline__ float sigmoid_fast(float z) {
  float t, r;
  asm("ex2.approx.ftz.f32 %0, %1;" : "=f"(t) : "f"(z * -1.4426950408889634f));
  asm("rcp.approx.ftz.f32 %0, %1;" : "=f"(r) : "f"(1.0f + t));
  return r;
}

__device__ __forceinline__ float erf_as(float z) {
  const float az = fabsf(z);
  const float t = __fdividef(1.0f, fmaf(0.3275911f, az, 1.0f));
  float poly = fmaf(1.061405429f, t, -1.453152027f);
  poly = fmaf(poly, t, 1.421413741f);
  poly = fmaf(poly, t, -0.284496736f);
  poly = fmaf(poly, t, 0.254829592f);
  poly *= t;
  const float e = exp2f(-az * az * 1.4426950408889634f);
  return copysignf(fmaf(-poly, e, 1.0f), z);
}
__device__ __forceinline__ float gelu_erf(float x) {
  return 0.5f * x * (1.0f + erf_as(x * 0.70710678118654752440f));
}

__device__ __forceinline__ float gelu_bf16_grade(float x) {
  const float xc = fminf(fmaxf(x, -4.5f), 4.5f);
  const float t = fmaf(xc * xc, 0.09876543209876543f, -1.0f);
  float p = -0.004680031910538673f;
  p = fmaf(p, t, 0.010336018167436123f);
  p = fmaf(p, t, -0.010503096505999565f);
  p = fmaf(p, t, 0.018587922677397728f);
  p = fmaf(p, t, -0.03804188221693039f);
  p = fmaf(p, t, 0.05810019373893738f);
  p = fmaf(p, t, -0.08021842688322067f);
  p = fmaf(p, t, 0.10921084135770798f);
  p = fmaf(p, t, -0.1543877273797989f);
  p = fmaf(p, t, 0.3138136863708496f);
  const float hx = 0.5f * x;
  return fmaf(hx, xc * p, hx);
}

__device__ __forceinline__ float ex2_approx(float x) {
  float y;
  asm("ex2.approx.ftz.f32 %0, %1;" : "=f"(y) : "f"(x));
  return y;
}

__device__ __forceinline__ float round_tf32(float x) {
  uint32_t r;
  asm("cvt.rna.tf32.f32 %0, %1;" : "=r"(r) : "f"(x));
  return __uint_as_float(r);
}

__device__ __forceinline__ uint32_t pack_bf16x2(float lo, float hi) {
  __nv_bfloat162 v = __floats2bfloat162_rn(lo, hi);
  return *reinterpret_cast<uint32_t*>(&v);
}

__device__ __forceinline__ unsigned long long globaltimer() {
  unsigned long long t;
  asm volatile("mov.u64 %0, %globaltimer;" : "=l"(t)::"memory");
  return t;
}

__device__ __forceinline__ uint32_t sw128_off(int row, int c) {
  return static_cast<uint32_t>(row * 128 + ((c ^ (row & 7)) << 4));
}

__device__ __forceinline__ void ldmatrix_x4(uint32_t (&r)[4], uint32_t addr) {
  asm volatile("ldmatrix.sync.aligned.m8n8.x4.shared.b16 {%0,%1,%2,%3}, [%4];"
               : "=r"(r[0]), "=r"(r[1]), "=r"(r[2]), "=r"(r[3])
               : "r"(addr));
}
__device__ __forceinline__ void ldmatrix_x4_trans(uint32_t (&r)[4], uint32_t addr) {
  asm volatile("ldmatrix.sync.aligned.m8n8.x4.trans.shared.b16 {%0,%1,%2,%3}, [%4];"
               : "=r"(r[0]), "=r"(r[1]), "=r"(r[2]), "=r"(r[3])
               : "r"(addr));
}
__device__ __forceinline__ void mma_bf16_16816(float (&c)[4], uint32_t a0, uint32_t a1, uint32_t a2, uint32_t a3,
                                               uint32_t b0, uint32_t b1) {
  asm volatile(
      "mma.sync.aligned.m16n8k16.row.col.f32.bf16.bf16.f32 {%0,%1,%2,%3}, {%4,%5,%6,%7}, {%8,%9}, {%0,%1,%2,%3};"
      : "+f"(c[0]), "+f"(c[1]), "+f"(c[2]), "+f"(c[3])
      : "r"(a0), "r"(a1), "r"(a2), "r"(a3), "r"(b0), "r"(b1));
}
__device__ __forceinline__ void mma_bf16_16816(float (&c)[4], const uint32_t (&a)[4], uint32_t b0, uint32_t b1) {
  mma_bf16_16816(c, a[0], a[1], a[2], a[3], b0, b1);
}

__device__ __forceinline__ void griddep_wait() { asm volatile("griddepcontrol.wait;" ::: "memory"); }
__device__ __forceinline__ void griddep_launch_dependents() { asm volatile("griddepcontrol.launch_dependents;" ::: "memory"); }

__device__ __forceinline__ void mbar_init(uint64_t* bar, uint32_t count) {
  asm volatile("mbarrier.init.shared::cta.b64 [%0], %1;" ::"r"(smem_u32(bar)), "r"(count) : "memory");
}
__device__ __forceinline__ void fence_mbar_init() {
  asm volatile("fence.mbarrier_init.release.cluster;" ::: "memory");
}
__device__ __forceinline__ void fence_proxy_async_smem() {
  asm volatile("fence.proxy.async.shared::cta;" ::: "memory");
}
__device__ __forceinline__ void mbar_arrive_expect_tx(uint64_t* bar, uint32_t bytes) {
  asm volatile("mbarrier.arrive.expect_tx.shared::cta.b64 _, [%0], %1;" ::"r"(smem_u32(bar)), "r"(bytes)
               : "memory");
}
__device__ __forceinline__ void mbar_arrive(uint64_t* bar) {
  asm volatile("mbarrier.arrive.shared::cta.b64 _, [%0];" ::"r"(smem_u32(bar)) : "memory");
}
__device__ __forceinline__ bool mbar_try_wait(uint64_t* bar, uint32_t parity) {
  uint32_t ok;
  asm volatile(
      "{\n\t.reg .pred p;\n\t"
      "mbarrier.try_wait.parity.shared::cta.b64 p, [%1], %2;\n\t"
      "selp.u32 %0, 1, 0, p;\n\t}"
      : "=r"(ok)
      : "r"(smem_u32(bar)), "r"(parity)
      : "memory");
  return ok != 0;
}
static __device__ __noinline__ void mbar_timeout(uint64_t* bar, uint32_t parity) {
  printf("avsep: mbarrier watchdog fired (block %d,%d thread %d, barrier at smem +%u, parity %u)\n", blockIdx.x, blockIdx.y,
         threadIdx.x, static_cast<unsigned>(__cvta_generic_to_shared(bar)), parity);
  __trap();
}
__device__ __forceinline__ void mbar_wait(uint64_t* bar, uint32_t parity) {
  if (mbar_try_wait(bar, parity)) return;
  const long long t0 = clock64();
  while (!mbar_try_wait(bar, parity)) {
    if (clock64() - t0 > AVSEP_WATCHDOG_CYCLES) mbar_timeout(bar, parity);
  }
}

__device__ __forceinline__ bool mbar_try_wait_hint(uint64_t* bar, uint32_t parity, uint32_t ns) {
  uint32_t ok;
  asm volatile(
      "{\n\t.reg .pred p;\n\t"
      "mbarrier.try_wait.parity.shared::cta.b64 p, [%1], %2, %3;\n\t"
      "selp.u32 %0, 1, 0, p;\n\t}"
      : "=r"(ok)
      : "r"(smem_u32(bar)), "r"(parity), "r"(ns)
      : "memory");
  return ok != 0;
}
__device__ __forceinline__ void mbar_wait_sleep(uint64_t* bar, uint32_t parity) {
  if (mbar_try_wait(bar, parity)) return;
  const long long t0 = clock64();
  while (!mbar_try_wait_hint(bar, parity, 1000u)) {
    if (clock64() - t0 > AVSEP_WATCHDOG_CYCLES) mbar_timeout(bar, parity);
  }
}

__device__ __forceinline__ void tma_prefetch_desc(const CUtensorMap* m) {
  asm volatile("prefetch.tensormap [%0];" ::"l"(reinterpret_cast<uint64_t>(m)) : "memory");
}
__device__ __forceinline__ void tma_load_2d(void* smem_dst, const CUtensorMap* m, uint64_t* bar, int c0, int c1) {
  asm volatile(
      "cp.async.bulk.tensor.2d.shared::cluster.global.mbarrier::complete_tx::bytes [%0], [%1, {%3, %4}], [%2];"
      ::"r"(smem_u32(smem_dst)), "l"(reinterpret_cast<uint64_t>(m)), "r"(smem_u32(bar)), "r"(c0), "r"(c1)
      : "memory");
}
__device__ __forceinline__ void tma_load_3d(void* smem_dst, const CUtensorMap* m, uint64_t* bar, int c0, int c1,
                                            int c2) {
  asm volatile(
      "cp.async.bulk.tensor.3d.shared::cluster.global.mbarrier::complete_tx::bytes [%0], [%1, {%3, %4, %5}], [%2];"
      ::"r"(smem_u32(smem_dst)), "l"(reinterpret_cast<uint64_t>(m)), "r"(smem_u32(bar)), "r"(c0), "r"(c1), "r"(c2)
      : "memory");
}

__device__ __forceinline__ void tma_store_2d(const CUtensorMap* m, const void* smem_src, int c0, int c1) {
  asm volatile("cp.async.bulk.tensor.2d.global.shared::cta.bulk_group [%0, {%2, %3}], [%1];"
               ::"l"(reinterpret_cast<uint64_t>(m)), "r"(smem_u32(smem_src)), "r"(c0), "r"(c1)
               : "memory");
}
__device__ __forceinline__ void bulk_commit() { asm volatile("cp.async.bulk.commit_group;" ::: "memory"); }
__device__ __forceinline__ void bulk_wait_read0() { asm volatile("cp.async.bulk.wait_group.read 0;" ::: "memory"); }
__device__ __forceinline__ void named_bar_sync(int id, int nthreads) {
  asm volatile("bar.sync %0, %1;" ::"r"(id), "r"(nthreads) : "memory");
}

__device__ __forceinline__ void tmem_alloc(uint32_t* smem_result, uint32_t ncols) {
  asm volatile("tcgen05.alloc.cta_group::1.sync.aligned.shared::cta.b32 [%0], %1;" ::"r"(smem_u32(smem_result)),
               "r"(ncols)
               : "memory");
  asm volatile("tcgen05.relinquish_alloc_permit.cta_group::1.sync.aligned;" ::: "memory");
}
__device__ __forceinline__ void tmem_dealloc(uint32_t taddr, uint32_t ncols) {
  asm volatile("tcgen05.dealloc.cta_group::1.sync.aligned.b32 %0, %1;" ::"r"(taddr), "r"(ncols) : "memory");
}
__device__ __forceinline__ void tc_fence_before() { asm volatile("tcgen05.fence::before_thread_sync;" ::: "memory"); }
__device__ __forceinline__ void tc_fence_after() { asm volatile("tcgen05.fence::after_thread_sync;" ::: "memory"); }

__device__ __forceinline__ void umma_f16(uint32_t d_tmem, uint64_t adesc, uint64_t bdesc, uint32_t idesc,
                                         uint32_t accumulate) {
  asm volatile(
      "{\n\t.reg .pred p;\n\t"
      "setp.ne.b32 p, %4, 0;\n\t"
      "tcgen05.mma.cta_group::1.kind::f16 [%0], %1, %2, %3, p;\n\t}"
      ::"r"(d_tmem), "l"(adesc), "l"(bdesc), "r"(idesc), "r"(accumulate)
      : "memory");
}
__device__ __forceinline__ void umma_tf32(uint32_t d_tmem, uint64_t adesc, uint64_t bdesc, uint32_t idesc,
                                          uint32_t accumulate) {
  asm volatile(
      "{\n\t.reg .pred p;\n\t"
      "setp.ne.b32 p, %4, 0;\n\t"
      "tcgen05.mma.cta_group::1.kind::tf32 [%0], %1, %2, %3, p;\n\t}"
      ::"r"(d_tmem), "l"(adesc), "l"(bdesc), "r"(idesc), "r"(accumulate)
      : "memory");
}
__device__ __forceinline__ void umma_f16_ts(uint32_t d_tmem, uint32_t a_tmem, uint64_t bdesc, uint32_t idesc,
                                            uint32_t accumulate) {
  asm volatile(
      "{\n\t.reg .pred p;\n\t"
      "setp.ne.b32 p, %4, 0;\n\t"
      "tcgen05.mma.cta_group::1.kind::f16 [%0], [%1], %2, %3, p;\n\t}"
      ::"r"(d_tmem), "r"(a_tmem), "l"(bdesc), "r"(idesc), "r"(accumulate)
      : "memory");
}
__device__ __forceinline__ void umma_commit(uint64_t* bar) {
  asm volatile("tcgen05.commit.cta_group::1.mbarrier::arrive::one.shared::cluster.b64 [%0];" ::"r"(smem_u32(bar))
               : "memory");
}
__device__ __forceinline__ void tmem_ld_wait() { asm volatile("tcgen05.wait::ld.sync.aligned;" ::: "memory"); }
__device__ __forceinline__ void tmem_st_wait() { asm volatile("tcgen05.wait::st.sync.aligned;" ::: "memory"); }

__device__ __forceinline__ void tmem_ld_32x32b_x32(uint32_t taddr, uint32_t (&r)[32]) {
  asm volatile(
      "tcgen05.ld.sync.aligned.32x32b.x32.b32 "
      "{%0, %1, %2, %3, %4, %5, %6, %7, %8, %9, %10, %11, %12, %13, %14, %15, "
      "%16, %17, %18, %19, %20, %21, %22, %23, %24, %25, %26, %27, %28, %29, %30, %31}, [%32];"
      : "=r"(r[0]), "=r"(r[1]), "=r"(r[2]), "=r"(r[3]), "=r"(r[4]), "=r"(r[5]), "=r"(r[6]), "=r"(r[7]),
        "=r"(r[8]), "=r"(r[9]), "=r"(r[10]), "=r"(r[11]), "=r"(r[12]), "=r"(r[13]), "=r"(r[14]), "=r"(r[15]),
        "=r"(r[16]), "=r"(r[17]), "=r"(r[18]), "=r"(r[19]), "=r"(r[20]), "=r"(r[21]), "=r"(r[22]), "=r"(r[23]),
        "=r"(r[24]), "=r"(r[25]), "=r"(r[26]), "=r"(r[27]), "=r"(r[28]), "=r"(r[29]), "=r"(r[30]), "=r"(r[31])
      : "r"(taddr)
      : "memory");
}

__device__ __forceinline__ void tmem_ld_32x32b_x16(uint32_t taddr, uint32_t (&r)[16]) {
  asm volatile(
      "tcgen05.ld.sync.aligned.32x32b.x16.b32 "
      "{%0, %1, %2, %3, %4, %5, %6, %7, %8, %9, %10, %11, %12, %13, %14, %15}, [%16];"
      : "=r"(r[0]), "=r"(r[1]), "=r"(r[2]), "=r"(r[3]), "=r"(r[4]), "=r"(r[5]), "=r"(r[6]), "=r"(r[7]),
        "=r"(r[8]), "=r"(r[9]), "=r"(r[10]), "=r"(r[11]), "=r"(r[12]), "=r"(r[13]), "=r"(r[14]), "=r"(r[15])
      : "r"(taddr)
      : "memory");
}

__device__ __forceinline__ void tmem_st_32x32b_x16(uint32_t taddr, const uint32_t (&r)[16]) {
  asm volatile(
      "tcgen05.st.sync.aligned.32x32b.x16.b32 [%0], "
      "{%1, %2, %3, %4, %5, %6, %7, %8, %9, %10, %11, %12, %13, %14, %15, %16};"
      ::"r"(taddr), "r"(r[0]), "r"(r[1]), "r"(r[2]), "r"(r[3]), "r"(r[4]), "r"(r[5]), "r"(r[6]), "r"(r[7]), "r"(r[8]),
        "r"(r[9]), "r"(r[10]), "r"(r[11]), "r"(r[12]), "r"(r[13]), "r"(r[14]), "r"(r[15])
      : "memory");
}

__device__ __forceinline__ void tmem_st_32x32b_x32(uint32_t taddr, const uint32_t (&r)[32]) {
  asm volatile(
      "tcgen05.st.sync.aligned.32x32b.x32.b32 [%0], "
      "{%1, %2, %3, %4, %5, %6, %7, %8, %9, %10, %11, %12, %13, %14, %15, %16, "
      "%17, %18, %19, %20, %21, %22, %23, %24, %25, %26, %27, %28, %29, %30, %31, %32};"
      ::"r"(taddr), "r"(r[0]), "r"(r[1]), "r"(r[2]), "r"(r[3]), "r"(r[4]), "r"(r[5]), "r"(r[6]), "r"(r[7]), "r"(r[8]),
        "r"(r[9]), "r"(r[10]), "r"(r[11]), "r"(r[12]), "r"(r[13]), "r"(r[14]), "r"(r[15]), "r"(r[16]), "r"(r[17]),
        "r"(r[18]), "r"(r[19]), "r"(r[20]), "r"(r[21]), "r"(r[22]), "r"(r[23]), "r"(r[24]), "r"(r[25]), "r"(r[26]),
        "r"(r[27]), "r"(r[28]), "r"(r[29]), "r"(r[30]), "r"(r[31])
      : "memory");
}

__device__ __forceinline__ uint64_t umma_desc_kmajor_sw128(uint32_t smem_addr, uint32_t sbo_bytes) {
  uint64_t d = 0;
  d |= static_cast<uint64_t>((smem_addr & 0x3FFFFu) >> 4);
  d |= static_cast<uint64_t>(1) << 16;
  d |= static_cast<uint64_t>((sbo_bytes >> 4) & 0x3FFFu) << 32;
  d |= static_cast<uint64_t>(1) << 46;
  d |= static_cast<uint64_t>(2) << 61;
  return d;
}
__device__ __forceinline__ uint64_t umma_desc_mnmajor_sw128(uint32_t smem_addr, uint32_t lbo_bytes,
                                                            uint32_t sbo_bytes) {
  uint64_t d = 0;
  d |= static_cast<uint64_t>((smem_addr & 0x3FFFFu) >> 4);
  d |= static_cast<uint64_t>((lbo_bytes >> 4) & 0x3FFFu) << 16;
  d |= static_cast<uint64_t>((sbo_bytes >> 4) & 0x3FFFu) << 32;
  d |= static_cast<uint64_t>(1) << 46;
  d |= static_cast<uint64_t>(2) << 61;
  return d;
}

__host__ __device__ constexpr uint32_t umma_idesc(uint32_t fmt, uint32_t M, uint32_t N, uint32_t a_mn = 0,
                                                  uint32_t b_mn = 0) {
  return (1u << 4) | (fmt << 7) | (fmt << 10) | (a_mn << 15) | (b_mn << 16) | ((N >> 3) << 17) | ((M >> 4) << 24);
}

}
```

av-separation-transformer_b200/csrc/kernels.h:

```cpp
#pragma once

#include <cuda.h>
#include <cuda_runtime.h>
#include <cuda_bf16.h>
#include <stdint.h>
#include <string.h>

namespace avsep {

inline uint16_t f2bf(float f) {
  uint32_t u;
  memcpy(&u, &f, 4);
  if ((u & 0x7fffffffu) > 0x7f800000u) return static_cast<uint16_t>((u >> 16) | 0x40);
  u += 0x7fffu + ((u >> 16) & 1u);
  return static_cast<uint16_t>(u >> 16);
}

const char* tma_init();
const char* tma_encode_2d(CUtensorMap* map, CUtensorMapDataType dt, int esz, const void* ptr, uint64_t inner,
                          uint64_t outer, uint64_t ld_elems, uint32_t box_inner, uint32_t box_outer);
const char* tma_encode_3d(CUtensorMap* map, CUtensorMapDataType dt, int esz, const void* ptr, uint64_t inner,
                          uint64_t outer, uint64_t batches, uint64_t ld_elems, uint32_t box_inner, uint32_t box_outer);
bool smem_opt_in(const void* kern, int bytes);
template <typename... KArgs>
bool smem_opt_in(void (*kern)(KArgs...), int bytes) {
  return smem_opt_in(reinterpret_cast<const void*>(kern), bytes);
}

void pdl_set(bool on);
bool pdl_enabled();
template <typename... KArgs, typename... Args>
inline cudaError_t launch_pdl(void (*kern)(KArgs...), dim3 grid, dim3 block, size_t smem, cudaStream_t s, Args... args) {
  cudaLaunchConfig_t cfg = {};
  cfg.gridDim = grid;
  cfg.blockDim = block;
  cfg.dynamicSmemBytes = smem;
  cfg.stream = s;
  cudaLaunchAttribute attr[1];
  attr[0].id = cudaLaunchAttributeProgrammaticStreamSerialization;
  attr[0].val.programmaticStreamSerializationAllowed = 1;
  cfg.attrs = attr;
  cfg.numAttrs = pdl_enabled() ? 1 : 0;
  return cudaLaunchKernelEx(&cfg, kern, KArgs(args)...);
}


enum Precision { PREC_BF16 = 0, PREC_TF32 = 1 };
enum Act { ACT_NONE = 0, ACT_RELU = 1, ACT_GELU = 2, ACT_GELU_BF16 = 3 };
enum RowMap { ROW_IDENT = 0, ROW_PAD2PAD = 1, ROW_PAD2COMPACT = 2 };
enum EpiKind { EPI_STD = 0, EPI_TAIL = 1, EPI_LN = 2, EPI_LN_TMA = 3 };

struct GemmProblem {
  const void* A;
  int lda;
  int rowsA;
  int M;
  const void* W;
  int ldw;
  int N;
  int K;
  int taps;
  int tap_stride;
  int row_shift;
};

struct GemmEpilogue {
  int kind = EPI_STD;
  const float* bias = nullptr;
  int act = ACT_NONE;
  int rowmap = ROW_IDENT;
  int Lp = 0;
  const float* pe = nullptr;
  int pe_period = 0;
  float* out_f32 = nullptr;
  int ld_f32 = 0;
  void* out_op = nullptr;
  int ld_op = 0;
  const float* resid = nullptr;
  const float* ln_gamma = nullptr;
  const float* ln_beta = nullptr;
  const float* mixed = nullptr;
  float* masks = nullptr;
  float* separated = nullptr;
  int F = 0, S = 0, T = 0;
  const int* lens = nullptr;
};
__device__ __forceinline__ int utt_len(const int* lens, int b, int L) {
  return lens == nullptr ? L : min(max(__ldg(lens + b), 1), L);
}
__device__ __forceinline__ bool frame_live(const int* lens, int N, int fr) {
  return lens == nullptr || fr % N < utt_len(lens, fr / N, N);
}

const char* launch_gemm(cudaStream_t s, int prec, const GemmProblem& p, const GemmEpilogue& e, int num_sms,
                        int force_bn = 0, unsigned long long* trace = nullptr);
bool gemm_ln_fusable(int N);

bool ffn_fusable(int prec, int d_model);
const char* launch_ffn_fused(cudaStream_t s, const void* a, const void* w1, const float* b1, const void* w2,
                             const float* b2, int act, const float* resid, float* x_out, const float* gamma,
                             const float* beta, void* out_op, int M, int num_sms,
                             unsigned long long* trace = nullptr);
struct StackProblem {
  const float* x_in;
  float* out_x;
  void* out_op;
  const float *fin_gamma, *fin_beta;
  const uint8_t* wstream;
  int n_layers;
  bool cross;
  const void* kv;
  int kv_ld;
  int B, L;
  int act;
  long long* trace = nullptr;
  const void* pro_a = nullptr;
  int pro_rows = 0, pro_pitch = 0, pro_taps = 0, pro_k = 0, pro_relu = 0;
  const float* pe = nullptr;
  void* kvp_out = nullptr;
  int kvp_L = 0, kvp_n = 0, kvp_ld = 0;
  const float* mixed = nullptr;
  float *masks = nullptr, *separated = nullptr;
  int F = 0, S = 0;
  const int* lens = nullptr;
  const int* kvp_lens = nullptr;
};
bool xformer_decoder_usable(int S, int F);
int xformer_decoder_chunks(int S, int F);
size_t xformer_decoder_bytes(int S, int F);
void xformer_pack_decoder(const float* w0, const float* b0, const float* w3, const float* b3, int S, int F, uint8_t* dst);
size_t xformer_pro_bytes(int taps, int K);
void xformer_pack_pro(const float* W, int ld, int col_stride, int taps, int K, uint8_t* dst);
bool xformer_kvp_usable(int n, int L_src, int L_out);
size_t xformer_kvp_bytes(int n);
void xformer_pack_kvp(const float* wkv, const float* bkv, int n, uint8_t* dst);
bool xformer_stack_usable(int prec, int d_model, int nhead, int len);
size_t xformer_stream_bytes(bool cross);
int xformer_vec_floats();
void xformer_pack_self(const float* wqkv, const float* wo, const float* w1, const float* w2, const float* vecs,
                       uint8_t* dst);
void xformer_pack_cross(const float* wq, const float* wo, const float* w1, const float* w2, const float* vecs,
                        uint8_t* dst);
void xformer_pack_vecs(const float* bqkv, int n_bqkv, const float* bo, const float* b1, const float* b2, const float* n1g,
                       const float* n1b, const float* n2g, const float* n2b, float* dst, const float* b0 = nullptr);
const char* launch_xformer_stack(cudaStream_t s, const StackProblem& p, int num_sms);

const char* launch_add_layernorm(cudaStream_t s, int prec, const float* x, const float* y, const float* gamma,
                                 const float* beta, float* x_out, void* out_op, int M, int d);

const char* launch_prep_audio(cudaStream_t s, int prec, const float* mixed, void* xp, int B, int F, int T, int Fp,
                              const int* lens = nullptr);

const char* launch_separate(cudaStream_t s, const float* masks, const float* mixed, float* out, long long B, int S,
                            int F, int T);
struct FlagSet {
  static constexpr int MAX = 16;
  unsigned* ptr[MAX];
  int n;
};
const char* launch_flag_signal(cudaStream_t s, const FlagSet& f, unsigned value);
const char* launch_flag_wait(cudaStream_t s, const FlagSet& f, unsigned value, double timeout_s);

struct AttnProblem {
  const void* q; int ldq;
  const void* k; const void* v;
  int ldkv;
  void* out; int ldo;
  int B, H, hd, Lq, Lk;
  int lerp_src;
  int tc_mode;
  const int* k_lens = nullptr;
  const int* src_lens = nullptr;
};
const char* launch_attention(cudaStream_t s, int prec, const AttnProblem& p);
bool attention_tc_usable(int prec, const AttnProblem& p);
bool attention_tc_wanted(int prec, const AttnProblem& p);
const char* launch_attention_tc(cudaStream_t s, const AttnProblem& p);
const char* launch_lerp_rows(cudaStream_t s, const float* src, int ld_src, int B, int nsrc, int L, int cols,
                             void* dst_bf16, int ld_dst, const int* src_lens = nullptr, const int* dst_lens = nullptr);

struct CnnWeights {
  const uint32_t* w1; const float* b1;
  const uint32_t* w2; const float* b2;
  const uint32_t* w3; const float* b3;
  const uint32_t *w1l, *w2l, *w3l;
};
const char* launch_visual_cnn(cudaStream_t s, int prec, const float* frames, int M, int H, int W, const CnnWeights& w,
                              void* pooled, int num_sms, const int* frame_lens = nullptr, int N = 1);
size_t visual_cnn_tc_w2_bytes();
size_t visual_cnn_tc_w3_bytes();
void visual_cnn_tc_pack(const float* w2, const float* w3, uint8_t* w2_slabs, uint8_t* w3_rows);
const char* launch_visual_cnn_tc(cudaStream_t s, const float* frames, int M, const CnnWeights& w, const uint8_t* w2_slabs,
                                 const uint8_t* w3_rows, void* pooled, int num_sms,
                                 unsigned long long* trace = nullptr, const int* frame_lens = nullptr, int N = 1);
size_t visual_cnn_pack_sizes(int which);
void visual_cnn_pack(const float* w1, const float* w2, const float* w3, uint32_t* p1, uint32_t* p2, uint32_t* p3,
                     bool lo_part = false);

struct SynthProblem {
  int B, S, n, nfft, hop, nf, Hh, Ww;
  double duration;
  const double *amps, *freqs, *phases;
  const float* noise;
  float* waves;
  float *mixed_spec, *lip_frames, *clean_specs;
};
const char* launch_synth(cudaStream_t s, const SynthProblem& p);
const char* launch_eval_snr(cudaStream_t s, const float* separated, const float* targets, const float* mixed, int B,
                            int S, int FT, double* input_snr, double* output_snr, int* best_perm, double* si_snr);

const char* launch_stft_complex(cudaStream_t s, const float* waves, const int* lengths, int B, int L, int nfft, int hop,
                                float* spec, float* mag, int* frame_lengths);
const char* fft512_init_tables();
const char* launch_stft512_synth(cudaStream_t s, const float* waves, int B, int S, int n, int hop, float* mixed_spec,
                                 float* clean_specs);
const char* launch_istft_masked(cudaStream_t s, const float* spec, const float* masks, const int* lengths, int B, int S,
                                int T, int nfft, int hop, int L, float* waves);

}
```

av-separation-transformer_b200/csrc/launch_util.cu:

```cuda
#include "kernels.h"

#include <cudaTypedefs.h>

#include <mutex>
#include <unordered_map>

namespace avsep {

namespace {

PFN_cuTensorMapEncodeTiled_v12000 g_encode = nullptr;

const char* encode(CUtensorMap* map, CUtensorMapDataType dt, uint32_t rank, const void* ptr, const cuuint64_t* dims,
                   const cuuint64_t* strides, const cuuint32_t* box) {
  if (g_encode == nullptr) return "tma: tma_init() has not run";
  if ((reinterpret_cast<uintptr_t>(ptr) & 15) != 0) return "tma: pointer not 16-byte aligned";
  if ((strides[0] & 15) != 0) return "tma: leading dimension not a multiple of 16 bytes";
  const cuuint32_t estr[3] = {1, 1, 1};
  if (g_encode(map, dt, rank, const_cast<void*>(ptr), dims, strides, box, estr, CU_TENSOR_MAP_INTERLEAVE_NONE,
               CU_TENSOR_MAP_SWIZZLE_128B, CU_TENSOR_MAP_L2_PROMOTION_L2_256B, CU_TENSOR_MAP_FLOAT_OOB_FILL_NONE) !=
      CUDA_SUCCESS)
    return "tma: cuTensorMapEncodeTiled failed";
  return nullptr;
}

}

const char* tma_init() {
  if (g_encode != nullptr) return nullptr;
  void* fn = nullptr;
  cudaDriverEntryPointQueryResult qres;
  if (cudaGetDriverEntryPoint("cuTensorMapEncodeTiled", &fn, cudaEnableDefault, &qres) != cudaSuccess ||
      qres != cudaDriverEntryPointSuccess || fn == nullptr)
    return "tma: cuTensorMapEncodeTiled entry point not found (driver too old?)";
  g_encode = reinterpret_cast<PFN_cuTensorMapEncodeTiled_v12000>(fn);
  return nullptr;
}

const char* tma_encode_2d(CUtensorMap* map, CUtensorMapDataType dt, int esz, const void* ptr, uint64_t inner,
                          uint64_t outer, uint64_t ld_elems, uint32_t box_inner, uint32_t box_outer) {
  const cuuint64_t dims[2] = {inner, outer};
  const cuuint64_t strides[1] = {ld_elems * esz};
  const cuuint32_t box[2] = {box_inner, box_outer};
  return encode(map, dt, 2, ptr, dims, strides, box);
}

const char* tma_encode_3d(CUtensorMap* map, CUtensorMapDataType dt, int esz, const void* ptr, uint64_t inner,
                          uint64_t outer, uint64_t batches, uint64_t ld_elems, uint32_t box_inner, uint32_t box_outer) {
  const cuuint64_t dims[3] = {inner, outer, batches};
  const cuuint64_t strides[2] = {ld_elems * esz, outer * ld_elems * esz};
  const cuuint32_t box[3] = {box_inner, box_outer, 1};
  return encode(map, dt, 3, ptr, dims, strides, box);
}

bool smem_opt_in(const void* kern, int bytes) {
  static std::mutex mu;
  static std::unordered_map<const void*, int> limit;
  std::lock_guard<std::mutex> lock(mu);
  int& cur = limit[kern];
  if (bytes <= 48 * 1024 || bytes <= cur) return true;
  if (cudaFuncSetAttribute(kern, cudaFuncAttributeMaxDynamicSharedMemorySize, bytes) != cudaSuccess) return false;
  cur = bytes;
  return true;
}

}
```

av-separation-transformer_b200/csrc/visual_cnn_tc.cu:

```cuda
#include "common.cuh"
#include "kernels.h"

#include <string.h>

namespace avsep {

namespace {

constexpr int TC_BUILDERS = 256;
constexpr int TC_THREADS = TC_BUILDERS + 64;
constexpr int W3S = 4;
constexpr int GROUP = 8;
constexpr int SLAB_BYTES = 128 * 128;
constexpr int W2_SLABS = 5, W2_SLAB_BYTES = 64 * 128;
constexpr int NSLOT = 6;
constexpr int OFF_W3 = 0;
constexpr int OFF_W2 = OFF_W3 + W3S * SLAB_BYTES;
constexpr int OFF_ACT2 = OFF_W2 + W2_SLABS * W2_SLAB_BYTES;
constexpr int OFF_ACT1 = OFF_ACT2 + GROUP * 64 * 128;
constexpr int OFF_IN = OFF_ACT1 + 2 * 256 * 64;
constexpr int OFF_MISC = OFF_IN + 2 * 34 * 34 * 4;
constexpr int TC_SMEM = OFF_MISC + 256 + 1024;
static_assert(TC_SMEM <= 227 * 1024, "visual_cnn_tc: shared memory budget exceeded");

struct CnnTcDev {
  const float* frames;
  __nv_bfloat16* pooled;
  const uint32_t* w1; const float* b1;
  const uint8_t* w2_slabs; const float* b2;
  const float* b3;
  int M, num_groups;
  const int* frame_lens;
  int N;
  unsigned long long* trace;
};

#define CTRACE(slot) do { if (p.trace != nullptr && tid == 0 && grp == static_cast<int>(blockIdx.x + gridDim.x)) \
    p.trace[blockIdx.x * 64 + (slot)] = globaltimer(); } while (0)

__device__ __forceinline__ int act1_chunk_off(int pixel, int c) {
  const int line = pixel >> 1;
  return line * 128 + ((((pixel & 1) << 2) | c) ^ (line & 7)) * 16;
}
__device__ __forceinline__ int act2_chunk_off(int pixel, int c) {
  return pixel * 128 + ((c ^ (pixel & 7)) * 16);
}

__global__ void __launch_bounds__(TC_THREADS, 1)
visual_cnn_tc_kernel(const __grid_constant__ CUtensorMap tmW3, const CnnTcDev p) {
  extern __shared__ __align__(1024) uint8_t smem_raw_cnn[];
  uint8_t* const smem = smem_raw_cnn;
  if ((smem_u32(smem) & 1023u) != 0) __trap();
  uint8_t* w3s = smem + OFF_W3;
  uint8_t* w2s = smem + OFF_W2;
  uint8_t* act2 = smem + OFF_ACT2;
  uint8_t* act1 = smem + OFF_ACT1;
  float* sIn = reinterpret_cast<float*>(smem + OFF_IN);
  uint64_t* ring_full = reinterpret_cast<uint64_t*>(smem + OFF_MISC);
  uint64_t* ring_free = ring_full + NSLOT;
  uint64_t* bar_acc = ring_free + NSLOT;
  uint64_t* bar_acc3 = bar_acc + 1;
  uint64_t* bar_w3 = bar_acc3 + 2;
  uint64_t* w3_free = bar_w3 + W3S;
  uint32_t* tmem_slot = reinterpret_cast<uint32_t*>(w3_free + W3S);

  const int tid = threadIdx.x, warp = tid >> 5, lane = tid & 31;

  for (int i = tid; i < W2_SLABS * W2_SLAB_BYTES / 16; i += TC_THREADS)
    reinterpret_cast<uint4*>(w2s)[i] = reinterpret_cast<const uint4*>(p.w2_slabs)[i];
  for (int i = tid; i < 2 * 34 * 34; i += TC_THREADS) sIn[i] = 0.f;
  if (tid == 0) {
    tma_prefetch_desc(&tmW3);
    for (int i = 0; i < NSLOT; ++i) {
      mbar_init(&ring_full[i], TC_BUILDERS / 32);
      mbar_init(&ring_free[i], 1);
    }
    mbar_init(bar_acc, 1);
    mbar_init(&bar_acc3[0], 1);
    mbar_init(&bar_acc3[1], 1);
    for (int i = 0; i < W3S; ++i) { mbar_init(&bar_w3[i], 1); mbar_init(&w3_free[i], 1); }
    fence_mbar_init();
  }
  if (warp == TC_BUILDERS / 32) tmem_alloc(tmem_slot, 512);
  fence_proxy_async_smem();
  tc_fence_before();
  __syncthreads();
  tc_fence_after();
  const uint32_t tmem_base = *tmem_slot;
  const uint32_t tmem_acc2 = tmem_base;
  const uint32_t tmem_acc3 = tmem_base + 64;
  const uint32_t tmem_ring = tmem_base + 320;
  griddep_launch_dependents();
  griddep_wait();

  if (warp == TC_BUILDERS / 32) {
    if (lane == 0) {
      const uint32_t idesc2 = umma_idesc(1u, 128, 64);
      const uint32_t idesc3 = umma_idesc(1u, 128, 128);
      uint32_t n_slab = 0, n_w3 = 0, lt = 0;
      for (int grp = blockIdx.x; grp < p.num_groups; grp += gridDim.x, ++lt) {
        for (int pair = 0; pair < GROUP / 2; ++pair) {
          for (int j = 0; j < W2_SLABS; ++j, ++n_slab) {
            const uint32_t slot = n_slab % NSLOT, use = n_slab / NSLOT;
            mbar_wait(&ring_full[slot], use & 1);
            tc_fence_after();
            const uint32_t a_t = tmem_ring + slot * 32;
            const uint64_t bdesc = umma_desc_kmajor_sw128(smem_u32(w2s + j * W2_SLAB_BYTES), 1024);
            const int ksteps = (j == W2_SLABS - 1) ? 2 : 4;
            for (int k = 0; k < ksteps; ++k)
              umma_f16_ts(tmem_acc2, a_t + 8 * k, bdesc + 2 * k, idesc2, (j | k) != 0 ? 1u : 0u);
            umma_commit(&ring_free[slot]);
            if (j == W2_SLABS - 1) umma_commit(bar_acc);
          }
        }
        for (int t = 0; t < 9; ++t, ++n_slab, ++n_w3) {
          const uint32_t slot = n_slab % NSLOT, use = n_slab / NSLOT;
          mbar_wait(&ring_full[slot], use & 1);
          const uint32_t ws = n_w3 % W3S;
          mbar_wait(&bar_w3[ws], (n_w3 / W3S) & 1);
          tc_fence_after();
          const uint32_t a_t = tmem_ring + slot * 32;
          const uint64_t bdesc = umma_desc_kmajor_sw128(smem_u32(w3s + ws * SLAB_BYTES), 1024);
#pragma unroll
          for (int k = 0; k < 4; ++k)
            umma_f16_ts(tmem_acc3 + (lt & 1) * 128, a_t + 8 * k, bdesc + 2 * k, idesc3, (t | k) != 0 ? 1u : 0u);
          umma_commit(&ring_free[slot]);
          umma_commit(&w3_free[ws]);
          if (t == 8) umma_commit(&bar_acc3[lt & 1]);
        }
      }
    }
  } else if (warp == TC_BUILDERS / 32 + 1) {
    if (lane == 0) {
      uint32_t n = 0;
      for (int grp = blockIdx.x; grp < p.num_groups; grp += gridDim.x) {
        for (int t = 0; t < 9; ++t, ++n) {
          const uint32_t ws = n % W3S, use = n / W3S;
          if (use > 0) mbar_wait(&w3_free[ws], (use - 1) & 1);
          mbar_arrive_expect_tx(&bar_w3[ws], SLAB_BYTES);
          tma_load_2d(w3s + ws * SLAB_BYTES, &tmW3, &bar_w3[ws], 0, t * 128);
        }
      }
    }
  } else {
    const int gid = lane >> 2, tig = lane & 3;
    uint32_t n_slab = 0;
    uint32_t acc_phase = 0;

    const int bq = warp & 3, bhh = warp >> 2;
    const int brow = bq * 32 + lane;
    const uint32_t ring_lane = tmem_ring + (static_cast<uint32_t>(bq * 32) << 16) + bhh * 16;
    int xo2[3], s02[3];
    bool vx2[3];
    const int y2 = (brow >> 3) & 7, f2 = brow >> 6;
#pragma unroll
    for (int kx = 0; kx < 3; ++kx) {
      const int xx = 2 * (brow & 7) + kx - 1;
      vx2[kx] = xx >= 0 && xx < 16;
      xo2[kx] = (xx >> 1) * 128;
      s02[kx] = (((xx & 1) << 2) ^ ((xx >> 1) & 7));
    }
    const int rowbase2 = (f2 * 256 + (2 * y2 - 1) * 16) * 64;
    const bool top2 = (y2 == 0);
    int xo3[3], s03[3];
    bool vx3[3];
    const int y3 = (brow >> 2) & 3;
    const bool top3 = (y3 == 0);
#pragma unroll
    for (int kx = 0; kx < 3; ++kx) {
      const int xx = 2 * (brow & 3) + kx - 1;
      vx3[kx] = xx >= 0 && xx < 8;
      xo3[kx] = xx * 128;
      s03[kx] = xx & 7;
    }
    const int rowbase3 = ((brow >> 4) * 64 + (2 * y3 - 1) * 8) * 128;

    uint32_t bw1[4][2];
    float bias1[4][2];
#pragma unroll
    for (int nt = 0; nt < 4; ++nt) {
      bw1[nt][0] = __ldg(p.w1 + nt * 64 + lane * 2);
      bw1[nt][1] = __ldg(p.w1 + nt * 64 + lane * 2 + 1);
      bias1[nt][0] = __ldg(p.b1 + nt * 8 + 2 * tig);
      bias1[nt][1] = __ldg(p.b1 + nt * 8 + 2 * tig + 1);
    }
    const int k0 = 2 * tig, k1 = 2 * tig + 1;
    const int off0 = (k0 / 3) * 34 + (k0 % 3), off1 = (k1 / 3) * 34 + (k1 % 3), off8 = 2 * 34 + 2;

    float4 pre[2];
    auto prefetch_pair = [&](int first_frame) {
#pragma unroll
      for (int i = 0; i < 2; ++i) {
        const int id = tid + TC_BUILDERS * i;
        const int f = id >> 8, rem = id & 255;
        const int fr = first_frame + f;
        pre[i] = make_float4(0.f, 0.f, 0.f, 0.f);
        if (fr < p.M && frame_live(p.frame_lens, p.N, fr)) pre[i] = __ldg(reinterpret_cast<const float4*>(p.frames + static_cast<size_t>(fr) * 1024) + rem);
      }
    };
    auto publish_slab = [&](uint32_t slot, const uint32_t (&cols)[16]) {
      tmem_st_32x32b_x16(ring_lane + slot * 32, cols);
      tmem_st_wait();
      tc_fence_before();
      __syncwarp();
      if (lane == 0) mbar_arrive(&ring_full[slot]);
    };
    auto conv2_epilogue = [&](int pair_idx) {
      mbar_wait(bar_acc, acc_phase);
      acc_phase ^= 1;
      tc_fence_after();
      const int q = warp & 3, hh = warp >> 2;
      const int r = q * 32 + lane;
      uint32_t v[32];
      tmem_ld_32x32b_x32(tmem_acc2 + (static_cast<uint32_t>(q * 32) << 16) + hh * 32, v);
      tmem_ld_wait();
      const int pixel = pair_idx * 128 + r;
#pragma unroll
      for (int ch = 0; ch < 4; ++ch) {
        uint4 u;
        const float4 ba = __ldg(reinterpret_cast<const float4*>(p.b2 + hh * 32 + ch * 8));
        const float4 bc = __ldg(reinterpret_cast<const float4*>(p.b2 + hh * 32 + ch * 8 + 4));
        u.x = pack_bf16x2(fmaxf(__uint_as_float(v[ch * 8 + 0]) + ba.x, 0.f), fmaxf(__uint_as_float(v[ch * 8 + 1]) + ba.y, 0.f));
        u.y = pack_bf16x2(fmaxf(__uint_as_float(v[ch * 8 + 2]) + ba.z, 0.f), fmaxf(__uint_as_float(v[ch * 8 + 3]) + ba.w, 0.f));
        u.z = pack_bf16x2(fmaxf(__uint_as_float(v[ch * 8 + 4]) + bc.x, 0.f), fmaxf(__uint_as_float(v[ch * 8 + 5]) + bc.y, 0.f));
        u.w = pack_bf16x2(fmaxf(__uint_as_float(v[ch * 8 + 6]) + bc.z, 0.f), fmaxf(__uint_as_float(v[ch * 8 + 7]) + bc.w, 0.f));
        *reinterpret_cast<uint4*>(act2 + act2_chunk_off(pixel, hh * 4 + ch)) = u;
      }
      tc_fence_before();
      named_bar_sync(1, TC_BUILDERS);
    };

    auto conv3_epilogue = [&](uint32_t g_lt, int g_frame0) {
      mbar_wait(&bar_acc3[g_lt & 1], (g_lt >> 1) & 1);
      tc_fence_after();
      {
        const int q = warp & 3, hh = warp >> 2;
        const int fr = g_frame0 + q * 2 + (lane >> 4);
#pragma unroll
        for (int cc = 0; cc < 2; ++cc) {
          uint32_t v[32];
          const int col0 = hh * 64 + cc * 32;
          tmem_ld_32x32b_x32(tmem_acc3 + (g_lt & 1) * 128 + (static_cast<uint32_t>(q * 32) << 16) + col0, v);
          tmem_ld_wait();
          float x[32];
#pragma unroll
          for (int jx = 0; jx < 32; ++jx) x[jx] = fmaxf(__uint_as_float(v[jx]) + __ldg(p.b3 + col0 + jx), 0.f);
#pragma unroll
          for (int jx = 0; jx < 16; ++jx) {
            const bool up = (lane & 8) != 0;
            const float send = up ? x[jx] : x[jx + 16];
            const float recv = __shfl_xor_sync(0xffffffffu, send, 8);
            x[jx] = (up ? x[jx + 16] : x[jx]) + recv;
          }
#pragma unroll
          for (int jx = 0; jx < 8; ++jx) {
            const bool up = (lane & 4) != 0;
            const float send = up ? x[jx] : x[jx + 8];
            const float recv = __shfl_xor_sync(0xffffffffu, send, 4);
            x[jx] = (up ? x[jx + 8] : x[jx]) + recv;
          }
#pragma unroll
          for (int jx = 0; jx < 4; ++jx) {
            const bool up = (lane & 2) != 0;
            const float send = up ? x[jx] : x[jx + 4];
            const float recv = __shfl_xor_sync(0xffffffffu, send, 2);
            x[jx] = (up ? x[jx + 4] : x[jx]) + recv;
          }
#pragma unroll
          for (int jx = 0; jx < 2; ++jx) {
            const bool up = (lane & 1) != 0;
            const float send = up ? x[jx] : x[jx + 2];
            const float recv = __shfl_xor_sync(0xffffffffu, send, 1);
            x[jx] = (up ? x[jx + 2] : x[jx]) + recv;
          }
          if (fr < p.M) {
            const int cbase = ((lane & 8) ? 16 : 0) + ((lane & 4) ? 8 : 0) + ((lane & 2) ? 4 : 0) + ((lane & 1) ? 2 : 0);
            *reinterpret_cast<uint32_t*>(p.pooled + static_cast<size_t>(fr) * 128 + col0 + cbase) =
                pack_bf16x2(x[0] * (1.f / 16.f), x[1] * (1.f / 16.f));
          }
        }
      }
      tc_fence_before();
    };
    prefetch_pair(blockIdx.x * GROUP);
    uint32_t lt = 0;
    int prev_frame0 = 0;

    for (int grp = blockIdx.x; grp < p.num_groups; grp += gridDim.x, ++lt) {
      const int frame0 = grp * GROUP;
      CTRACE(0);
      for (int pair = 0; pair < GROUP / 2; ++pair) {
#pragma unroll
        for (int i = 0; i < 2; ++i) {
          const int id = tid + TC_BUILDERS * i;
          const int f = id >> 8, rem = id & 255;
          const int y = rem >> 3, x4 = (rem & 7) * 4;
          float* d = sIn + f * 34 * 34 + (y + 1) * 34 + (x4 + 1);
          d[0] = pre[i].x; d[1] = pre[i].y; d[2] = pre[i].z; d[3] = pre[i].w;
        }
        named_bar_sync(1, TC_BUILDERS);
        CTRACE(1 + pair * 5);
        {
          const int next_first = (pair + 1 < GROUP / 2) ? frame0 + (pair + 1) * 2 : (grp + static_cast<int>(gridDim.x)) * GROUP;
          prefetch_pair(next_first);
        }

#pragma unroll
        for (int t = warp; t < 32; t += TC_BUILDERS / 32) {
          uint32_t a[4] = {0, 0, 0, 0};
          int pix[2];
#pragma unroll
          for (int hf = 0; hf < 2; ++hf) {
            const int r = t * 16 + gid + 8 * hf;
            const int f = r >> 8, rem = r & 255, y = rem >> 4, x = rem & 15;
            pix[hf] = r;
            const float* base = sIn + f * 34 * 34 + (2 * y) * 34 + 2 * x;
            a[hf] = pack_bf16x2(base[off0], base[off1]);
            if (tig == 0) a[2 + hf] = pack_bf16x2(base[off8], 0.f);
          }
#pragma unroll
          for (int nt = 0; nt < 4; ++nt) {
            float cacc[4] = {0.f, 0.f, 0.f, 0.f};
            mma_bf16_16816(cacc, a[0], a[1], a[2], a[3], bw1[nt][0], bw1[nt][1]);
            const float bb0 = bias1[nt][0], bb1 = bias1[nt][1];
            *reinterpret_cast<uint32_t*>(act1 + act1_chunk_off(pix[0], nt) + tig * 4) =
                pack_bf16x2(fmaxf(cacc[0] + bb0, 0.f), fmaxf(cacc[1] + bb1, 0.f));
            *reinterpret_cast<uint32_t*>(act1 + act1_chunk_off(pix[1], nt) + tig * 4) =
                pack_bf16x2(fmaxf(cacc[2] + bb0, 0.f), fmaxf(cacc[3] + bb1, 0.f));
          }
        }
        named_bar_sync(1, TC_BUILDERS);
        CTRACE(2 + pair * 5);

        if (pair > 0) conv2_epilogue(pair - 1);
        if (pair == 1 && lt > 0) conv3_epilogue(lt - 1, prev_frame0);
        CTRACE(3 + pair * 5);

        for (int j = 0; j < W2_SLABS; ++j, ++n_slab) {
          const uint32_t slot = n_slab % NSLOT, use = n_slab / NSLOT;
          if (use > 0) mbar_wait(&ring_free[slot], (use - 1) & 1);
          const int tap = 2 * j + bhh;
          const int ky = (tap * 11) >> 5, kx = tap - 3 * ky;
          const bool ok = (tap < 9) && (kx == 0 ? vx2[0] : (kx == 1 ? vx2[1] : vx2[2])) && !(ky == 0 && top2);
          const int src = rowbase2 + ky * 1024 + (kx == 0 ? xo2[0] : (kx == 1 ? xo2[1] : xo2[2]));
          const int s0 = kx == 0 ? s02[0] : (kx == 1 ? s02[1] : s02[2]);
          uint32_t cols[16];
#pragma unroll
          for (int cch = 0; cch < 4; ++cch) {
            uint4 val = make_uint4(0, 0, 0, 0);
            if (ok) val = *reinterpret_cast<const uint4*>(act1 + src + ((s0 ^ cch) << 4));
            cols[4 * cch] = val.x; cols[4 * cch + 1] = val.y; cols[4 * cch + 2] = val.z; cols[4 * cch + 3] = val.w;
          }
          tc_fence_after();
          publish_slab(slot, cols);
        }
        CTRACE(4 + pair * 5);
      }
      conv2_epilogue(GROUP / 2 - 1);
      CTRACE(21);

      for (int t = 0; t < 9; ++t, ++n_slab) {
        const uint32_t slot = n_slab % NSLOT, use = n_slab / NSLOT;
        if (use > 0) mbar_wait(&ring_free[slot], (use - 1) & 1);
        const int ky = (t * 11) >> 5, kx = t - 3 * ky;
        const bool ok = (kx == 0 ? vx3[0] : (kx == 1 ? vx3[1] : vx3[2])) && !(ky == 0 && top3);
        const int src = rowbase3 + ky * 1024 + (kx == 0 ? xo3[0] : (kx == 1 ? xo3[1] : xo3[2]));
        const int s0 = kx == 0 ? s03[0] : (kx == 1 ? s03[1] : s03[2]);
        uint32_t cols[16];
#pragma unroll
        for (int cch = 0; cch < 4; ++cch) {
          uint4 val = make_uint4(0, 0, 0, 0);
          if (ok) val = *reinterpret_cast<const uint4*>(act2 + src + (((4 * bhh + cch) ^ s0) << 4));
          cols[4 * cch] = val.x; cols[4 * cch + 1] = val.y; cols[4 * cch + 2] = val.z; cols[4 * cch + 3] = val.w;
        }
        tc_fence_after();
        publish_slab(slot, cols);
      }
      CTRACE(22);
      CTRACE(23);
      CTRACE(24);
      prev_frame0 = frame0;
    }
    if (lt > 0) conv3_epilogue(lt - 1, prev_frame0);
  }

  tc_fence_before();
  __syncthreads();
  if (warp == TC_BUILDERS / 32) {
    tc_fence_after();
    tmem_dealloc(tmem_base, 512);
  }
}

}

size_t visual_cnn_tc_w2_bytes() { return W2_SLABS * W2_SLAB_BYTES; }
size_t visual_cnn_tc_w3_bytes() { return 9 * SLAB_BYTES; }

void visual_cnn_tc_pack(const float* w2, const float* w3, uint8_t* w2_slabs, uint8_t* w3_rows) {
  memset(w2_slabs, 0, visual_cnn_tc_w2_bytes());
  for (int j = 0; j < W2_SLABS; ++j)
    for (int n = 0; n < 64; ++n)
      for (int k = 0; k < 64; ++k) {
        const int tap = 2 * j + (k >> 5), c = k & 31;
        const float val = tap < 9 ? w2[static_cast<size_t>(n) * 288 + tap * 32 + c] : 0.f;
        const int chunk = (k >> 3) ^ (n & 7);
        uint16_t* dst = reinterpret_cast<uint16_t*>(w2_slabs + j * W2_SLAB_BYTES + n * 128 + chunk * 16) + (k & 7);
        *dst = f2bf(val);
      }
  uint16_t* o = reinterpret_cast<uint16_t*>(w3_rows);
  for (int t = 0; t < 9; ++t)
    for (int n = 0; n < 128; ++n)
      for (int c = 0; c < 64; ++c) o[(static_cast<size_t>(t) * 128 + n) * 64 + c] = f2bf(w3[static_cast<size_t>(n) * 576 + t * 64 + c]);
}

const char* launch_visual_cnn_tc(cudaStream_t s, const float* frames, int M, const CnnWeights& w, const uint8_t* w2_slabs,
                                 const uint8_t* w3_rows, void* pooled, int num_sms, unsigned long long* trace,
                                 const int* frame_lens, int N) {
  if (M <= 0) return "visual_cnn_tc: empty problem";
  CUtensorMap tm;
  if (const char* e = tma_encode_2d(&tm, CU_TENSOR_MAP_DATA_TYPE_BFLOAT16, 2, w3_rows, 64, 9 * 128, 64, 64, 128)) return e;
  if (!smem_opt_in(visual_cnn_tc_kernel, TC_SMEM)) return "visual_cnn_tc: cudaFuncSetAttribute failed";
  CnnTcDev d;
  d.frames = frames; d.pooled = reinterpret_cast<__nv_bfloat16*>(pooled);
  d.w1 = w.w1; d.b1 = w.b1; d.w2_slabs = w2_slabs; d.b2 = w.b2; d.b3 = w.b3;
  d.M = M; d.num_groups = (M + GROUP - 1) / GROUP;
  d.trace = trace;
  d.frame_lens = frame_lens; d.N = N;
  const int grid = d.num_groups < num_sms ? d.num_groups : num_sms;
  launch_pdl(visual_cnn_tc_kernel, dim3(grid), dim3(TC_THREADS), TC_SMEM, s, tm, d);
  return cudaGetLastError() == cudaSuccess ? nullptr : "visual_cnn_tc: launch failed";
}

}
```

Before: 481,500.

## Build conv2/conv3 A operands with TMA im2col from global scratch activations

The visual CNN tensor-core kernel used to have builder warps gather im2col slabs for conv2 and conv3 from shared memory into a ring. It now writes conv1 and conv2 activations to per-CTA global scratch in NHWC layout and uses dedicated im2col warps issuing TMA im2col loads into an A-slab ring. Extra mbarrier stages and a deeper epilogue lag with more TMEM accumulator buffers decouple the stages. The aim is to take operand-gather work off the builder warps and overlap the stages. In exchange, activations now make a round trip through global memory and L2, the kernel needs workspace scratch and async-proxy fences, and the pipeline is more complex.

```diff
diff --git a/av-separation-transformer_b200/csrc/avsep_api.cu b/av-separation-transformer_b200/csrc/avsep_api.cu
--- a/av-separation-transformer_b200/csrc/avsep_api.cu
+++ b/av-separation-transformer_b200/csrc/avsep_api.cu
@@ -80,6 +80,7 @@
   void *pooled, *v_op, *qkv_v, *attn_v, *ffn_v;
   float *x_v, *y_v, *kvn;
   void* kvb;
+  void* cnn_scratch;
 };
 
 }
@@ -114,6 +115,8 @@
   bool xs_v_kvp = false;
   void* own_ws = nullptr;
   size_t own_ws_bytes = 0;
+  void* cnn_test_scratch = nullptr;
+  size_t cnn_test_scratch_bytes = 0;
   struct HostSlot {
     float* io[4] = {nullptr, nullptr, nullptr, nullptr};
     size_t cap[4] = {0, 0, 0, 0};
@@ -192,6 +195,10 @@
 
 size_t op_size(const avsep_handle* h) { return h->cfg.precision == AVSEP_PREC_TF32 ? 4 : 2; }
 
+bool cnn_tc_selected(const avsep_handle* h, int Hh, int Ww) {
+  return Hh == 32 && Ww == 32 && h->cfg.precision == AVSEP_PREC_BF16;
+}
+
 size_t carve_workspace(const avsep_handle* h, Workspace& w, uint8_t* base, int B, int T, int N, int Hh, int Ww) {
   const size_t d = h->cfg.d_model, os = op_size(h);
   const size_t Ma = static_cast<size_t>(B) * T, Map = static_cast<size_t>(B) * (T + 2), Mv = static_cast<size_t>(B) * N;
@@ -219,6 +226,7 @@
   w.ffn_v = take(Mv * 4 * d * os);
   w.kvn = static_cast<float*>(take(Mv * h->cfg.num_fusion_layers * 2 * d * 4));
   w.kvb = take(Ma * h->cfg.num_fusion_layers * 2 * d * os);
+  w.cnn_scratch = take(cnn_tc_selected(h, Hh, Ww) ? visual_cnn_tc_scratch_bytes(static_cast<int>(Mv), h->num_sms) : 0);
   w.bytes = off;
   return off;
 }
@@ -272,9 +280,9 @@
 }
 
 const char* run_visual_cnn(avsep_handle* h, cudaStream_t s, const float* frames, int M, int Hh, int Ww, void* pooled,
-                           unsigned long long* trace = nullptr, const int* frame_lens = nullptr, int N = 1) {
-  if (Hh == 32 && Ww == 32 && h->cfg.precision == AVSEP_PREC_BF16)
-    return launch_visual_cnn_tc(s, frames, M, h->cnn, h->cnn_w2_slabs, h->cnn_w3_rows, pooled, h->num_sms, trace,
+                           void* scratch, unsigned long long* trace = nullptr, const int* frame_lens = nullptr, int N = 1) {
+  if (cnn_tc_selected(h, Hh, Ww))
+    return launch_visual_cnn_tc(s, frames, M, h->cnn, h->cnn_w2_slabs, h->cnn_w3_rows, pooled, scratch, h->num_sms, trace,
                                 frame_lens, N);
   return launch_visual_cnn(s, h->cfg.precision, frames, M, Hh, Ww, h->cnn, pooled, h->num_sms, frame_lens, N);
 }
@@ -447,7 +455,7 @@
   h->prof_stream = s;
   const int d = h->cfg.d_model, B = w.B, N = w.N;
   const int Mv = B * N;
-  CKL("visual_cnn", run_visual_cnn(h, s, frames, Mv, w.Hh, w.Ww, w.pooled, nullptr, w.frame_lens, N));
+  CKL("visual_cnn", run_visual_cnn(h, s, frames, Mv, w.Hh, w.Ww, w.pooled, w.cnn_scratch, nullptr, w.frame_lens, N));
   if (snapshot(h, s, "visual_pool", w.pooled, static_cast<size_t>(Mv) * 128, true)) return 1;
   if (pl.stack_v && pl.pro) return 0;
   const GemmProblem p = dense(w.pooled, Mv, 128, h->wproj, d);
@@ -724,6 +732,22 @@
                     t.n1g->data.data(), t.n1b->data.data(), t.n2g->data.data(), t.n2b->data.data(), vecs.data(), b0);
   (cross ? xformer_pack_cross : xformer_pack_self)(t.w_in->data.data(), t.wo->data.data(), t.w1->data.data(),
                                                    t.w2->data.data(), vecs.data(), dst);
+}
+
+int test_visual_cnn(avsep_handle* h, const float* frames, int M, int Hh, int Ww, void* pooled, unsigned long long* trace,
+                    cudaStream_t s) {
+  if (!h) return 1;
+  if (!h->finalized) return fail(h, "weights not finalized");
+  const size_t need = cnn_tc_selected(h, Hh, Ww) && M > 0 ? visual_cnn_tc_scratch_bytes(M, h->num_sms) : 0;
+  if (need > h->cnn_test_scratch_bytes) {
+    if (h->cnn_test_scratch) { cudaDeviceSynchronize(); cudaFree(h->cnn_test_scratch); }
+    h->cnn_test_scratch = nullptr;
+    h->cnn_test_scratch_bytes = 0;
+    CUDA_OK(cudaMalloc(&h->cnn_test_scratch, need));
+    h->cnn_test_scratch_bytes = need;
+  }
+  CK(run_visual_cnn(h, s, frames, M, Hh, Ww, pooled, h->cnn_test_scratch, trace));
+  return 0;
 }
 
 }
@@ -780,6 +804,7 @@
   cudaSetDevice(h->cfg.device);
   if (h->d_weights) cudaFree(h->d_weights);
   if (h->own_ws) cudaFree(h->own_ws);
+  if (h->cnn_test_scratch) cudaFree(h->cnn_test_scratch);
   for (auto& sl : h->slot) {
     for (float* ptr : sl.io)
       if (ptr) cudaFree(ptr);
@@ -1607,18 +1632,12 @@
 
 int avsep_test_visual_cnn(avsep_handle* h, const float* frames, int32_t M, int32_t Hh, int32_t Ww, void* pooled,
                           void* cuda_stream) {
-  if (!h) return 1;
-  if (!h->finalized) return fail(h, "weights not finalized");
-  CK(run_visual_cnn(h, static_cast<cudaStream_t>(cuda_stream), frames, M, Hh, Ww, pooled));
-  return 0;
+  return test_visual_cnn(h, frames, M, Hh, Ww, pooled, nullptr, static_cast<cudaStream_t>(cuda_stream));
 }
 
 int avsep_test_visual_cnn_trace(avsep_handle* h, const float* frames, int32_t M, void* pooled,
                                 unsigned long long* trace_dev, void* cuda_stream) {
-  if (!h) return 1;
-  if (!h->finalized) return fail(h, "weights not finalized");
-  CK(run_visual_cnn(h, static_cast<cudaStream_t>(cuda_stream), frames, M, 32, 32, pooled, trace_dev));
-  return 0;
-}
-
-}
+  return test_visual_cnn(h, frames, M, 32, 32, pooled, trace_dev, static_cast<cudaStream_t>(cuda_stream));
+}
+
+}
diff --git a/av-separation-transformer_b200/csrc/common.cuh b/av-separation-transformer_b200/csrc/common.cuh
--- a/av-separation-transformer_b200/csrc/common.cuh
+++ b/av-separation-transformer_b200/csrc/common.cuh
@@ -121,6 +121,9 @@
 __device__ __forceinline__ void fence_proxy_async_smem() {
   asm volatile("fence.proxy.async.shared::cta;" ::: "memory");
 }
+__device__ __forceinline__ void fence_proxy_async_global() {
+  asm volatile("fence.proxy.async.global;" ::: "memory");
+}
 __device__ __forceinline__ void mbar_arrive_expect_tx(uint64_t* bar, uint32_t bytes) {
   asm volatile("mbarrier.arrive.expect_tx.shared::cta.b64 _, [%0], %1;" ::"r"(smem_u32(bar)), "r"(bytes)
                : "memory");
@@ -185,6 +188,15 @@
   asm volatile(
       "cp.async.bulk.tensor.3d.shared::cluster.global.mbarrier::complete_tx::bytes [%0], [%1, {%3, %4, %5}], [%2];"
       ::"r"(smem_u32(smem_dst)), "l"(reinterpret_cast<uint64_t>(m)), "r"(smem_u32(bar)), "r"(c0), "r"(c1), "r"(c2)
+      : "memory");
+}
+__device__ __forceinline__ void tma_load_im2col_4d(void* smem_dst, const CUtensorMap* m, uint64_t* bar, int c, int w,
+                                                   int h, int n, uint16_t ow, uint16_t oh) {
+  asm volatile(
+      "cp.async.bulk.tensor.4d.shared::cluster.global.im2col.mbarrier::complete_tx::bytes"
+      " [%0], [%1, {%3, %4, %5, %6}], [%2], {%7, %8};"
+      ::"r"(smem_u32(smem_dst)), "l"(reinterpret_cast<uint64_t>(m)), "r"(smem_u32(bar)), "r"(c), "r"(w), "r"(h), "r"(n),
+        "h"(ow), "h"(oh)
       : "memory");
 }
 
@@ -296,6 +308,15 @@
   d |= static_cast<uint64_t>((sbo_bytes >> 4) & 0x3FFFu) << 32;
   d |= static_cast<uint64_t>(1) << 46;
   d |= static_cast<uint64_t>(2) << 61;
+  return d;
+}
+__device__ __forceinline__ uint64_t umma_desc_kmajor_sw64(uint32_t smem_addr, uint32_t sbo_bytes) {
+  uint64_t d = 0;
+  d |= static_cast<uint64_t>((smem_addr & 0x3FFFFu) >> 4);
+  d |= static_cast<uint64_t>(1) << 16;
+  d |= static_cast<uint64_t>((sbo_bytes >> 4) & 0x3FFFu) << 32;
+  d |= static_cast<uint64_t>(1) << 46;
+  d |= static_cast<uint64_t>(4) << 61;
   return d;
 }
 __device__ __forceinline__ uint64_t umma_desc_mnmajor_sw128(uint32_t smem_addr, uint32_t lbo_bytes,
diff --git a/av-separation-transformer_b200/csrc/kernels.h b/av-separation-transformer_b200/csrc/kernels.h
--- a/av-separation-transformer_b200/csrc/kernels.h
+++ b/av-separation-transformer_b200/csrc/kernels.h
@@ -21,6 +21,8 @@
                           uint64_t outer, uint64_t ld_elems, uint32_t box_inner, uint32_t box_outer);
 const char* tma_encode_3d(CUtensorMap* map, CUtensorMapDataType dt, int esz, const void* ptr, uint64_t inner,
                           uint64_t outer, uint64_t batches, uint64_t ld_elems, uint32_t box_inner, uint32_t box_outer);
+const char* tma_encode_im2col(CUtensorMap* map, const void* ptr, uint32_t c, uint32_t w, uint32_t h, uint64_t n,
+                              uint32_t stride, uint32_t pixels, CUtensorMapSwizzle swizzle);
 bool smem_opt_in(const void* kern, int bytes);
 template <typename... KArgs>
 bool smem_opt_in(void (*kern)(KArgs...), int bytes) {
@@ -189,9 +191,10 @@
                               void* pooled, int num_sms, const int* frame_lens = nullptr, int N = 1);
 size_t visual_cnn_tc_w2_bytes();
 size_t visual_cnn_tc_w3_bytes();
+size_t visual_cnn_tc_scratch_bytes(int M, int num_sms);
 void visual_cnn_tc_pack(const float* w2, const float* w3, uint8_t* w2_slabs, uint8_t* w3_rows);
 const char* launch_visual_cnn_tc(cudaStream_t s, const float* frames, int M, const CnnWeights& w, const uint8_t* w2_slabs,
-                                 const uint8_t* w3_rows, void* pooled, int num_sms,
+                                 const uint8_t* w3_rows, void* pooled, void* scratch, int num_sms,
                                  unsigned long long* trace = nullptr, const int* frame_lens = nullptr, int N = 1);
 size_t visual_cnn_pack_sizes(int which);
 void visual_cnn_pack(const float* w1, const float* w2, const float* w3, uint32_t* p1, uint32_t* p2, uint32_t* p3,
diff --git a/av-separation-transformer_b200/csrc/launch_util.cu b/av-separation-transformer_b200/csrc/launch_util.cu
--- a/av-separation-transformer_b200/csrc/launch_util.cu
+++ b/av-separation-transformer_b200/csrc/launch_util.cu
@@ -10,6 +10,7 @@
 namespace {
 
 PFN_cuTensorMapEncodeTiled_v12000 g_encode = nullptr;
+PFN_cuTensorMapEncodeIm2col_v12000 g_encode_im2col = nullptr;
 
 const char* encode(CUtensorMap* map, CUtensorMapDataType dt, uint32_t rank, const void* ptr, const cuuint64_t* dims,
                    const cuuint64_t* strides, const cuuint32_t* box) {
@@ -33,7 +34,12 @@
   if (cudaGetDriverEntryPoint("cuTensorMapEncodeTiled", &fn, cudaEnableDefault, &qres) != cudaSuccess ||
       qres != cudaDriverEntryPointSuccess || fn == nullptr)
     return "tma: cuTensorMapEncodeTiled entry point not found (driver too old?)";
+  void* fn2 = nullptr;
+  if (cudaGetDriverEntryPoint("cuTensorMapEncodeIm2col", &fn2, cudaEnableDefault, &qres) != cudaSuccess ||
+      qres != cudaDriverEntryPointSuccess || fn2 == nullptr)
+    return "tma: cuTensorMapEncodeIm2col entry point not found (driver too old?)";
   g_encode = reinterpret_cast<PFN_cuTensorMapEncodeTiled_v12000>(fn);
+  g_encode_im2col = reinterpret_cast<PFN_cuTensorMapEncodeIm2col_v12000>(fn2);
   return nullptr;
 }
 
@@ -53,6 +59,23 @@
   return encode(map, dt, 3, ptr, dims, strides, box);
 }
 
+const char* tma_encode_im2col(CUtensorMap* map, const void* ptr, uint32_t c, uint32_t w, uint32_t h, uint64_t n,
+                              uint32_t stride, uint32_t pixels, CUtensorMapSwizzle swizzle) {
+  if (g_encode_im2col == nullptr) return "tma: tma_init() has not run";
+  if ((reinterpret_cast<uintptr_t>(ptr) & 15) != 0) return "tma: pointer not 16-byte aligned";
+  if ((c * 2) % 16 != 0) return "tma: pixel row not a multiple of 16 bytes";
+  const cuuint64_t dims[4] = {c, w, h, n};
+  const cuuint64_t strides[3] = {static_cast<cuuint64_t>(c) * 2, static_cast<cuuint64_t>(c) * 2 * w,
+                                 static_cast<cuuint64_t>(c) * 2 * w * h};
+  const int lower[2] = {-1, -1}, upper[2] = {-1, -1};
+  const cuuint32_t estr[4] = {1, stride, stride, 1};
+  if (g_encode_im2col(map, CU_TENSOR_MAP_DATA_TYPE_BFLOAT16, 4, const_cast<void*>(ptr), dims, strides, lower, upper, c,
+                      pixels, estr, CU_TENSOR_MAP_INTERLEAVE_NONE, swizzle, CU_TENSOR_MAP_L2_PROMOTION_L2_128B,
+                      CU_TENSOR_MAP_FLOAT_OOB_FILL_NONE) != CUDA_SUCCESS)
+    return "tma: cuTensorMapEncodeIm2col failed";
+  return nullptr;
+}
+
 bool smem_opt_in(const void* kern, int bytes) {
   static std::mutex mu;
   static std::unordered_map<const void*, int> limit;
diff --git a/av-separation-transformer_b200/csrc/visual_cnn_tc.cu b/av-separation-transformer_b200/csrc/visual_cnn_tc.cu
--- a/av-separation-transformer_b200/csrc/visual_cnn_tc.cu
+++ b/av-separation-transformer_b200/csrc/visual_cnn_tc.cu
@@ -8,19 +8,25 @@
 namespace {
 
 constexpr int TC_BUILDERS = 256;
-constexpr int TC_THREADS = TC_BUILDERS + 64;
+constexpr int IM2COL_WARPS = 2;
+constexpr int TC_THREADS = TC_BUILDERS + 32 * (2 + IM2COL_WARPS);
+constexpr int MMA_WARP = TC_BUILDERS / 32, W3_WARP = MMA_WARP + 1, IM2COL_WARP = MMA_WARP + 2;
 constexpr int W3S = 4;
 constexpr int GROUP = 8;
 constexpr int SLAB_BYTES = 128 * 128;
 constexpr int W2_SLABS = 5, W2_SLAB_BYTES = 64 * 128;
-constexpr int NSLOT = 6;
+constexpr int NA = 6;
+constexpr int A1S = 3;
+constexpr int A2S = 2;
+constexpr int EPI_LAG = 2, ACC2_BUFS = 4;
+static_assert(EPI_LAG >= 1 && EPI_LAG < GROUP / 2 && ACC2_BUFS > EPI_LAG && ACC2_BUFS * 64 + 256 <= 512, "visual_cnn_tc: TMEM columns");
+constexpr int ACT1_FRAME_BYTES = 16 * 16 * 32 * 2, ACT2_FRAME_BYTES = 8 * 8 * 64 * 2;
 constexpr int OFF_W3 = 0;
 constexpr int OFF_W2 = OFF_W3 + W3S * SLAB_BYTES;
-constexpr int OFF_ACT2 = OFF_W2 + W2_SLABS * W2_SLAB_BYTES;
-constexpr int OFF_ACT1 = OFF_ACT2 + GROUP * 64 * 128;
-constexpr int OFF_IN = OFF_ACT1 + 2 * 256 * 64;
+constexpr int OFF_A = OFF_W2 + W2_SLABS * W2_SLAB_BYTES;
+constexpr int OFF_IN = OFF_A + NA * SLAB_BYTES;
 constexpr int OFF_MISC = OFF_IN + 2 * 34 * 34 * 4;
-constexpr int TC_SMEM = OFF_MISC + 256 + 1024;
+constexpr int TC_SMEM = OFF_MISC + 512 + 1024;
 static_assert(TC_SMEM <= 227 * 1024, "visual_cnn_tc: shared memory budget exceeded");
 
 struct CnnTcDev {
@@ -29,6 +35,8 @@
   const uint32_t* w1; const float* b1;
   const uint8_t* w2_slabs; const float* b2;
   const float* b3;
+  uint8_t* act1;
+  uint8_t* act2;
   int M, num_groups;
   const int* frame_lens;
   int N;
@@ -38,28 +46,38 @@
 #define CTRACE(slot) do { if (p.trace != nullptr && tid == 0 && grp == static_cast<int>(blockIdx.x + gridDim.x)) \
     p.trace[blockIdx.x * 64 + (slot)] = globaltimer(); } while (0)
 
-__device__ __forceinline__ int act1_chunk_off(int pixel, int c) {
-  const int line = pixel >> 1;
-  return line * 128 + ((((pixel & 1) << 2) | c) ^ (line & 7)) * 16;
-}
-__device__ __forceinline__ int act2_chunk_off(int pixel, int c) {
-  return pixel * 128 + ((c ^ (pixel & 7)) * 16);
+__device__ __forceinline__ void quad_transpose(uint32_t (&x)[4], int t) {
+  const bool odd = (t & 1) != 0, hi = (t & 2) != 0;
+#pragma unroll
+  for (int k = 0; k < 4; k += 2) {
+    const uint32_t r = __shfl_xor_sync(0xffffffffu, odd ? x[k] : x[k + 1], 1);
+    if (odd) x[k] = r; else x[k + 1] = r;
+  }
+#pragma unroll
+  for (int k = 0; k < 2; ++k) {
+    const uint32_t r = __shfl_xor_sync(0xffffffffu, hi ? x[k] : x[k + 2], 2);
+    if (hi) x[k] = r; else x[k + 2] = r;
+  }
 }
 
 __global__ void __launch_bounds__(TC_THREADS, 1)
-visual_cnn_tc_kernel(const __grid_constant__ CUtensorMap tmW3, const CnnTcDev p) {
+visual_cnn_tc_kernel(const __grid_constant__ CUtensorMap tmW3, const __grid_constant__ CUtensorMap tmA1,
+                     const __grid_constant__ CUtensorMap tmA2, const CnnTcDev p) {
   extern __shared__ __align__(1024) uint8_t smem_raw_cnn[];
   uint8_t* const smem = smem_raw_cnn;
   if ((smem_u32(smem) & 1023u) != 0) __trap();
   uint8_t* w3s = smem + OFF_W3;
   uint8_t* w2s = smem + OFF_W2;
-  uint8_t* act2 = smem + OFF_ACT2;
-  uint8_t* act1 = smem + OFF_ACT1;
+  uint8_t* as = smem + OFF_A;
   float* sIn = reinterpret_cast<float*>(smem + OFF_IN);
-  uint64_t* ring_full = reinterpret_cast<uint64_t*>(smem + OFF_MISC);
-  uint64_t* ring_free = ring_full + NSLOT;
-  uint64_t* bar_acc = ring_free + NSLOT;
-  uint64_t* bar_acc3 = bar_acc + 1;
+  uint64_t* a_full = reinterpret_cast<uint64_t*>(smem + OFF_MISC);
+  uint64_t* a_free = a_full + NA;
+  uint64_t* act1_full = a_free + NA;
+  uint64_t* act1_free = act1_full + A1S;
+  uint64_t* act2_full = act1_free + A1S;
+  uint64_t* act2_free = act2_full + A2S;
+  uint64_t* bar_acc2 = act2_free + A2S;
+  uint64_t* bar_acc3 = bar_acc2 + ACC2_BUFS;
   uint64_t* bar_w3 = bar_acc3 + 2;
   uint64_t* w3_free = bar_w3 + W3S;
   uint32_t* tmem_slot = reinterpret_cast<uint32_t*>(w3_free + W3S);
@@ -71,66 +89,72 @@
   for (int i = tid; i < 2 * 34 * 34; i += TC_THREADS) sIn[i] = 0.f;
   if (tid == 0) {
     tma_prefetch_desc(&tmW3);
-    for (int i = 0; i < NSLOT; ++i) {
-      mbar_init(&ring_full[i], TC_BUILDERS / 32);
-      mbar_init(&ring_free[i], 1);
-    }
-    mbar_init(bar_acc, 1);
-    mbar_init(&bar_acc3[0], 1);
-    mbar_init(&bar_acc3[1], 1);
+    tma_prefetch_desc(&tmA1);
+    tma_prefetch_desc(&tmA2);
+    for (int i = 0; i < NA; ++i) { mbar_init(&a_full[i], 1); mbar_init(&a_free[i], 1); }
+    for (int i = 0; i < A1S; ++i) { mbar_init(&act1_full[i], TC_BUILDERS / 32); mbar_init(&act1_free[i], 1); }
+    for (int i = 0; i < A2S; ++i) { mbar_init(&act2_full[i], TC_BUILDERS / 32); mbar_init(&act2_free[i], 1); }
+    for (int i = 0; i < ACC2_BUFS; ++i) mbar_init(&bar_acc2[i], 1);
+    for (int i = 0; i < 2; ++i) mbar_init(&bar_acc3[i], 1);
     for (int i = 0; i < W3S; ++i) { mbar_init(&bar_w3[i], 1); mbar_init(&w3_free[i], 1); }
     fence_mbar_init();
   }
-  if (warp == TC_BUILDERS / 32) tmem_alloc(tmem_slot, 512);
+  if (warp == MMA_WARP) tmem_alloc(tmem_slot, 512);
   fence_proxy_async_smem();
   tc_fence_before();
   __syncthreads();
   tc_fence_after();
   const uint32_t tmem_base = *tmem_slot;
   const uint32_t tmem_acc2 = tmem_base;
-  const uint32_t tmem_acc3 = tmem_base + 64;
-  const uint32_t tmem_ring = tmem_base + 320;
+  const uint32_t tmem_acc3 = tmem_base + ACC2_BUFS * 64;
+  const int act1_frame0 = blockIdx.x * A1S * 2, act2_frame0 = blockIdx.x * A2S * GROUP;
   griddep_launch_dependents();
   griddep_wait();
 
-  if (warp == TC_BUILDERS / 32) {
+  if (warp == MMA_WARP) {
     if (lane == 0) {
       const uint32_t idesc2 = umma_idesc(1u, 128, 64);
       const uint32_t idesc3 = umma_idesc(1u, 128, 128);
-      uint32_t n_slab = 0, n_w3 = 0, lt = 0;
-      for (int grp = blockIdx.x; grp < p.num_groups; grp += gridDim.x, ++lt) {
-        for (int pair = 0; pair < GROUP / 2; ++pair) {
-          for (int j = 0; j < W2_SLABS; ++j, ++n_slab) {
-            const uint32_t slot = n_slab % NSLOT, use = n_slab / NSLOT;
-            mbar_wait(&ring_full[slot], use & 1);
-            tc_fence_after();
-            const uint32_t a_t = tmem_ring + slot * 32;
-            const uint64_t bdesc = umma_desc_kmajor_sw128(smem_u32(w2s + j * W2_SLAB_BYTES), 1024);
-            const int ksteps = (j == W2_SLABS - 1) ? 2 : 4;
-            for (int k = 0; k < ksteps; ++k)
-              umma_f16_ts(tmem_acc2, a_t + 8 * k, bdesc + 2 * k, idesc2, (j | k) != 0 ? 1u : 0u);
-            umma_commit(&ring_free[slot]);
-            if (j == W2_SLABS - 1) umma_commit(bar_acc);
-          }
-        }
-        for (int t = 0; t < 9; ++t, ++n_slab, ++n_w3) {
-          const uint32_t slot = n_slab % NSLOT, use = n_slab / NSLOT;
-          mbar_wait(&ring_full[slot], use & 1);
+      uint32_t na = 0, n_w3 = 0, npair = 0, lt = 0;
+      auto conv3_group = [&](uint32_t g) {
+        for (int t = 0; t < 9; ++t, ++na, ++n_w3) {
+          const uint32_t slot = na % NA;
+          mbar_wait(&a_full[slot], (na / NA) & 1);
           const uint32_t ws = n_w3 % W3S;
           mbar_wait(&bar_w3[ws], (n_w3 / W3S) & 1);
           tc_fence_after();
-          const uint32_t a_t = tmem_ring + slot * 32;
+          if (t == 8) mbar_arrive(&act2_free[g % A2S]);
+          const uint64_t adesc = umma_desc_kmajor_sw128(smem_u32(as + slot * SLAB_BYTES), 1024);
           const uint64_t bdesc = umma_desc_kmajor_sw128(smem_u32(w3s + ws * SLAB_BYTES), 1024);
 #pragma unroll
           for (int k = 0; k < 4; ++k)
-            umma_f16_ts(tmem_acc3 + (lt & 1) * 128, a_t + 8 * k, bdesc + 2 * k, idesc3, (t | k) != 0 ? 1u : 0u);
-          umma_commit(&ring_free[slot]);
+            umma_f16(tmem_acc3 + (g & 1) * 128, adesc + 2 * k, bdesc + 2 * k, idesc3, (t | k) != 0 ? 1u : 0u);
+          umma_commit(&a_free[slot]);
           umma_commit(&w3_free[ws]);
-          if (t == 8) umma_commit(&bar_acc3[lt & 1]);
-        }
-      }
+          if (t == 8) umma_commit(&bar_acc3[g & 1]);
+        }
+      };
+      for (int grp = blockIdx.x; grp < p.num_groups; grp += gridDim.x, ++lt) {
+        for (int pair = 0; pair < GROUP / 2; ++pair, ++npair) {
+          if (pair == EPI_LAG && lt > 0) conv3_group(lt - 1);
+          const uint32_t acc = tmem_acc2 + (npair % ACC2_BUFS) * 64;
+          for (int t = 0; t < 9; ++t, ++na) {
+            const uint32_t slot = na % NA;
+            mbar_wait(&a_full[slot], (na / NA) & 1);
+            tc_fence_after();
+            if (t == 8) mbar_arrive(&act1_free[npair % A1S]);
+            const uint64_t adesc = umma_desc_kmajor_sw64(smem_u32(as + slot * SLAB_BYTES), 512);
+            const uint64_t bdesc = umma_desc_kmajor_sw128(smem_u32(w2s + (t >> 1) * W2_SLAB_BYTES), 1024) + (t & 1) * 4;
+#pragma unroll
+            for (int k = 0; k < 2; ++k) umma_f16(acc, adesc + 2 * k, bdesc + 2 * k, idesc2, (t | k) != 0 ? 1u : 0u);
+            umma_commit(&a_free[slot]);
+          }
+          umma_commit(&bar_acc2[npair % ACC2_BUFS]);
+        }
+      }
+      if (lt > 0) conv3_group(lt - 1);
     }
-  } else if (warp == TC_BUILDERS / 32 + 1) {
+  } else if (warp == W3_WARP) {
     if (lane == 0) {
       uint32_t n = 0;
       for (int grp = blockIdx.x; grp < p.num_groups; grp += gridDim.x) {
@@ -142,38 +166,35 @@
         }
       }
     }
+  } else if (warp >= IM2COL_WARP) {
+    if (lane == 0) {
+      const uint32_t me = warp - IM2COL_WARP;
+      uint32_t na = 0, npair = 0, lt = 0;
+      auto load_tap = [&](const CUtensorMap* tm, int frame, int t, uint32_t bytes) {
+        if (na++ % IM2COL_WARPS != me) return;
+        const uint32_t slot = (na - 1) % NA, use = (na - 1) / NA;
+        if (use > 0) mbar_wait(&a_free[slot], (use - 1) & 1);
+        mbar_arrive_expect_tx(&a_full[slot], bytes);
+        tma_load_im2col_4d(as + slot * SLAB_BYTES, tm, &a_full[slot], 0, -1, -1, frame, static_cast<uint16_t>(t % 3),
+                           static_cast<uint16_t>(t / 3));
+      };
+      auto conv3_group = [&](uint32_t g) {
+        const uint32_t s2 = g % A2S;
+        mbar_wait(&act2_full[s2], (g / A2S) & 1);
+        for (int t = 0; t < 9; ++t) load_tap(&tmA2, act2_frame0 + s2 * GROUP, t, SLAB_BYTES);
+      };
+      for (int grp = blockIdx.x; grp < p.num_groups; grp += gridDim.x, ++lt) {
+        for (int pair = 0; pair < GROUP / 2; ++pair, ++npair) {
+          if (pair == EPI_LAG && lt > 0) conv3_group(lt - 1);
+          const uint32_t s1 = npair % A1S;
+          mbar_wait(&act1_full[s1], (npair / A1S) & 1);
+          for (int t = 0; t < 9; ++t) load_tap(&tmA1, act1_frame0 + s1 * 2, t, 128 * 64);
+        }
+      }
+      if (lt > 0) conv3_group(lt - 1);
+    }
   } else {
     const int gid = lane >> 2, tig = lane & 3;
-    uint32_t n_slab = 0;
-    uint32_t acc_phase = 0;
-
-    const int bq = warp & 3, bhh = warp >> 2;
-    const int brow = bq * 32 + lane;
-    const uint32_t ring_lane = tmem_ring + (static_cast<uint32_t>(bq * 32) << 16) + bhh * 16;
-    int xo2[3], s02[3];
-    bool vx2[3];
-    const int y2 = (brow >> 3) & 7, f2 = brow >> 6;
-#pragma unroll
-    for (int kx = 0; kx < 3; ++kx) {
-      const int xx = 2 * (brow & 7) + kx - 1;
-      vx2[kx] = xx >= 0 && xx < 16;
-      xo2[kx] = (xx >> 1) * 128;
-      s02[kx] = (((xx & 1) << 2) ^ ((xx >> 1) & 7));
-    }
-    const int rowbase2 = (f2 * 256 + (2 * y2 - 1) * 16) * 64;
-    const bool top2 = (y2 == 0);
-    int xo3[3], s03[3];
-    bool vx3[3];
-    const int y3 = (brow >> 2) & 3;
-    const bool top3 = (y3 == 0);
-#pragma unroll
-    for (int kx = 0; kx < 3; ++kx) {
-      const int xx = 2 * (brow & 3) + kx - 1;
-      vx3[kx] = xx >= 0 && xx < 8;
-      xo3[kx] = xx * 128;
-      s03[kx] = xx & 7;
-    }
-    const int rowbase3 = ((brow >> 4) * 64 + (2 * y3 - 1) * 8) * 128;
 
     uint32_t bw1[4][2];
     float bias1[4][2];
@@ -198,23 +219,20 @@
         if (fr < p.M && frame_live(p.frame_lens, p.N, fr)) pre[i] = __ldg(reinterpret_cast<const float4*>(p.frames + static_cast<size_t>(fr) * 1024) + rem);
       }
     };
-    auto publish_slab = [&](uint32_t slot, const uint32_t (&cols)[16]) {
-      tmem_st_32x32b_x16(ring_lane + slot * 32, cols);
-      tmem_st_wait();
-      tc_fence_before();
+    auto publish = [&](uint64_t* bar) {
+      fence_proxy_async_global();
       __syncwarp();
-      if (lane == 0) mbar_arrive(&ring_full[slot]);
+      if (lane == 0) mbar_arrive(bar);
     };
-    auto conv2_epilogue = [&](int pair_idx) {
-      mbar_wait(bar_acc, acc_phase);
-      acc_phase ^= 1;
+    auto conv2_epilogue = [&](uint32_t np, int pair_idx, uint32_t s2) {
+      mbar_wait(&bar_acc2[np % ACC2_BUFS], (np / ACC2_BUFS) & 1);
       tc_fence_after();
       const int q = warp & 3, hh = warp >> 2;
       const int r = q * 32 + lane;
       uint32_t v[32];
-      tmem_ld_32x32b_x32(tmem_acc2 + (static_cast<uint32_t>(q * 32) << 16) + hh * 32, v);
+      tmem_ld_32x32b_x32(tmem_acc2 + (np % ACC2_BUFS) * 64 + (static_cast<uint32_t>(q * 32) << 16) + hh * 32, v);
       tmem_ld_wait();
-      const int pixel = pair_idx * 128 + r;
+      uint4* dst = reinterpret_cast<uint4*>(p.act2 + (static_cast<size_t>(act2_frame0 + s2 * GROUP) * 64 + pair_idx * 128 + r) * 128 + hh * 64);
 #pragma unroll
       for (int ch = 0; ch < 4; ++ch) {
         uint4 u;
@@ -224,13 +242,13 @@
         u.y = pack_bf16x2(fmaxf(__uint_as_float(v[ch * 8 + 2]) + ba.z, 0.f), fmaxf(__uint_as_float(v[ch * 8 + 3]) + ba.w, 0.f));
         u.z = pack_bf16x2(fmaxf(__uint_as_float(v[ch * 8 + 4]) + bc.x, 0.f), fmaxf(__uint_as_float(v[ch * 8 + 5]) + bc.y, 0.f));
         u.w = pack_bf16x2(fmaxf(__uint_as_float(v[ch * 8 + 6]) + bc.z, 0.f), fmaxf(__uint_as_float(v[ch * 8 + 7]) + bc.w, 0.f));
-        *reinterpret_cast<uint4*>(act2 + act2_chunk_off(pixel, hh * 4 + ch)) = u;
+        dst[ch] = u;
       }
       tc_fence_before();
-      named_bar_sync(1, TC_BUILDERS);
     };
 
-    auto conv3_epilogue = [&](uint32_t g_lt, int g_frame0) {
+    auto conv3_epilogue = [&](uint32_t g_lt) {
+      const int g_frame0 = (blockIdx.x + g_lt * gridDim.x) * GROUP;
       mbar_wait(&bar_acc3[g_lt & 1], (g_lt >> 1) & 1);
       tc_fence_after();
       {
@@ -282,14 +300,20 @@
       }
       tc_fence_before();
     };
+    auto finish_pair = [&](uint32_t np) {
+      const uint32_t g = np / (GROUP / 2), s2 = g % A2S;
+      const int pair_idx = np % (GROUP / 2);
+      if (pair_idx == 0 && g >= A2S) mbar_wait(&act2_free[s2], (g / A2S - 1) & 1);
+      conv2_epilogue(np, pair_idx, s2);
+      if (pair_idx == GROUP / 2 - 1) publish(&act2_full[s2]);
+    };
     prefetch_pair(blockIdx.x * GROUP);
-    uint32_t lt = 0;
-    int prev_frame0 = 0;
+    uint32_t lt = 0, npair = 0;
 
     for (int grp = blockIdx.x; grp < p.num_groups; grp += gridDim.x, ++lt) {
       const int frame0 = grp * GROUP;
       CTRACE(0);
-      for (int pair = 0; pair < GROUP / 2; ++pair) {
+      for (int pair = 0; pair < GROUP / 2; ++pair, ++npair) {
 #pragma unroll
         for (int i = 0; i < 2; ++i) {
           const int id = tid + TC_BUILDERS * i;
@@ -299,12 +323,15 @@
           d[0] = pre[i].x; d[1] = pre[i].y; d[2] = pre[i].z; d[3] = pre[i].w;
         }
         named_bar_sync(1, TC_BUILDERS);
-        CTRACE(1 + pair * 5);
+        CTRACE(1 + pair * 3);
         {
           const int next_first = (pair + 1 < GROUP / 2) ? frame0 + (pair + 1) * 2 : (grp + static_cast<int>(gridDim.x)) * GROUP;
           prefetch_pair(next_first);
         }
 
+        const uint32_t s1 = npair % A1S;
+        if (npair >= A1S) mbar_wait(&act1_free[s1], (npair / A1S - 1) & 1);
+        uint8_t* act1 = p.act1 + static_cast<size_t>(act1_frame0 + s1 * 2) * ACT1_FRAME_BYTES;
 #pragma unroll
         for (int t = warp; t < 32; t += TC_BUILDERS / 32) {
           uint32_t a[4] = {0, 0, 0, 0};
@@ -318,75 +345,37 @@
             a[hf] = pack_bf16x2(base[off0], base[off1]);
             if (tig == 0) a[2 + hf] = pack_bf16x2(base[off8], 0.f);
           }
+          uint32_t o[2][4];
 #pragma unroll
           for (int nt = 0; nt < 4; ++nt) {
             float cacc[4] = {0.f, 0.f, 0.f, 0.f};
             mma_bf16_16816(cacc, a[0], a[1], a[2], a[3], bw1[nt][0], bw1[nt][1]);
             const float bb0 = bias1[nt][0], bb1 = bias1[nt][1];
-            *reinterpret_cast<uint32_t*>(act1 + act1_chunk_off(pix[0], nt) + tig * 4) =
-                pack_bf16x2(fmaxf(cacc[0] + bb0, 0.f), fmaxf(cacc[1] + bb1, 0.f));
-            *reinterpret_cast<uint32_t*>(act1 + act1_chunk_off(pix[1], nt) + tig * 4) =
-                pack_bf16x2(fmaxf(cacc[2] + bb0, 0.f), fmaxf(cacc[3] + bb1, 0.f));
-          }
-        }
+            o[0][nt] = pack_bf16x2(fmaxf(cacc[0] + bb0, 0.f), fmaxf(cacc[1] + bb1, 0.f));
+            o[1][nt] = pack_bf16x2(fmaxf(cacc[2] + bb0, 0.f), fmaxf(cacc[3] + bb1, 0.f));
+          }
+#pragma unroll
+          for (int hf = 0; hf < 2; ++hf) {
+            quad_transpose(o[hf], tig);
+            *reinterpret_cast<uint4*>(act1 + pix[hf] * 64 + tig * 16) = make_uint4(o[hf][0], o[hf][1], o[hf][2], o[hf][3]);
+          }
+        }
+        publish(&act1_full[s1]);
         named_bar_sync(1, TC_BUILDERS);
-        CTRACE(2 + pair * 5);
-
-        if (pair > 0) conv2_epilogue(pair - 1);
-        if (pair == 1 && lt > 0) conv3_epilogue(lt - 1, prev_frame0);
-        CTRACE(3 + pair * 5);
-
-        for (int j = 0; j < W2_SLABS; ++j, ++n_slab) {
-          const uint32_t slot = n_slab % NSLOT, use = n_slab / NSLOT;
-          if (use > 0) mbar_wait(&ring_free[slot], (use - 1) & 1);
-          const int tap = 2 * j + bhh;
-          const int ky = (tap * 11) >> 5, kx = tap - 3 * ky;
-          const bool ok = (tap < 9) && (kx == 0 ? vx2[0] : (kx == 1 ? vx2[1] : vx2[2])) && !(ky == 0 && top2);
-          const int src = rowbase2 + ky * 1024 + (kx == 0 ? xo2[0] : (kx == 1 ? xo2[1] : xo2[2]));
-          const int s0 = kx == 0 ? s02[0] : (kx == 1 ? s02[1] : s02[2]);
-          uint32_t cols[16];
-#pragma unroll
-          for (int cch = 0; cch < 4; ++cch) {
-            uint4 val = make_uint4(0, 0, 0, 0);
-            if (ok) val = *reinterpret_cast<const uint4*>(act1 + src + ((s0 ^ cch) << 4));
-            cols[4 * cch] = val.x; cols[4 * cch + 1] = val.y; cols[4 * cch + 2] = val.z; cols[4 * cch + 3] = val.w;
-          }
-          tc_fence_after();
-          publish_slab(slot, cols);
-        }
-        CTRACE(4 + pair * 5);
-      }
-      conv2_epilogue(GROUP / 2 - 1);
-      CTRACE(21);
-
-      for (int t = 0; t < 9; ++t, ++n_slab) {
-        const uint32_t slot = n_slab % NSLOT, use = n_slab / NSLOT;
-        if (use > 0) mbar_wait(&ring_free[slot], (use - 1) & 1);
-        const int ky = (t * 11) >> 5, kx = t - 3 * ky;
-        const bool ok = (kx == 0 ? vx3[0] : (kx == 1 ? vx3[1] : vx3[2])) && !(ky == 0 && top3);
-        const int src = rowbase3 + ky * 1024 + (kx == 0 ? xo3[0] : (kx == 1 ? xo3[1] : xo3[2]));
-        const int s0 = kx == 0 ? s03[0] : (kx == 1 ? s03[1] : s03[2]);
-        uint32_t cols[16];
-#pragma unroll
-        for (int cch = 0; cch < 4; ++cch) {
-          uint4 val = make_uint4(0, 0, 0, 0);
-          if (ok) val = *reinterpret_cast<const uint4*>(act2 + src + (((4 * bhh + cch) ^ s0) << 4));
-          cols[4 * cch] = val.x; cols[4 * cch + 1] = val.y; cols[4 * cch + 2] = val.z; cols[4 * cch + 3] = val.w;
-        }
-        tc_fence_after();
-        publish_slab(slot, cols);
-      }
-      CTRACE(22);
-      CTRACE(23);
-      CTRACE(24);
-      prev_frame0 = frame0;
+        CTRACE(2 + pair * 3);
+
+        if (npair >= EPI_LAG) finish_pair(npair - EPI_LAG);
+        if (pair == GROUP / 2 - 1 && lt > 0) conv3_epilogue(lt - 1);
+        CTRACE(3 + pair * 3);
+      }
     }
-    if (lt > 0) conv3_epilogue(lt - 1, prev_frame0);
+    for (uint32_t np = npair >= EPI_LAG ? npair - EPI_LAG : 0; np < npair; ++np) finish_pair(np);
+    if (lt > 0) conv3_epilogue(lt - 1);
   }
 
   tc_fence_before();
   __syncthreads();
-  if (warp == TC_BUILDERS / 32) {
+  if (warp == MMA_WARP) {
     tc_fence_after();
     tmem_dealloc(tmem_base, 512);
   }
@@ -396,6 +385,14 @@
 
 size_t visual_cnn_tc_w2_bytes() { return W2_SLABS * W2_SLAB_BYTES; }
 size_t visual_cnn_tc_w3_bytes() { return 9 * SLAB_BYTES; }
+
+static int cnn_tc_grid(int M, int num_sms) {
+  const int groups = (M + GROUP - 1) / GROUP;
+  return groups < num_sms ? groups : num_sms;
+}
+size_t visual_cnn_tc_scratch_bytes(int M, int num_sms) {
+  return static_cast<size_t>(cnn_tc_grid(M, num_sms)) * (A1S * 2 * ACT1_FRAME_BYTES + A2S * GROUP * ACT2_FRAME_BYTES);
+}
 
 void visual_cnn_tc_pack(const float* w2, const float* w3, uint8_t* w2_slabs, uint8_t* w3_rows) {
   memset(w2_slabs, 0, visual_cnn_tc_w2_bytes());
@@ -415,20 +412,30 @@
 }
 
 const char* launch_visual_cnn_tc(cudaStream_t s, const float* frames, int M, const CnnWeights& w, const uint8_t* w2_slabs,
-                                 const uint8_t* w3_rows, void* pooled, int num_sms, unsigned long long* trace,
-                                 const int* frame_lens, int N) {
+                                 const uint8_t* w3_rows, void* pooled, void* scratch, int num_sms,
+                                 unsigned long long* trace, const int* frame_lens, int N) {
   if (M <= 0) return "visual_cnn_tc: empty problem";
-  CUtensorMap tm;
+  if (scratch == nullptr) return "visual_cnn_tc: no scratch (visual_cnn_tc_scratch_bytes)";
+  const int grid = cnn_tc_grid(M, num_sms);
+  uint8_t* act1 = static_cast<uint8_t*>(scratch);
+  uint8_t* act2 = act1 + static_cast<size_t>(grid) * A1S * 2 * ACT1_FRAME_BYTES;
+  CUtensorMap tm, tm1, tm2;
   if (const char* e = tma_encode_2d(&tm, CU_TENSOR_MAP_DATA_TYPE_BFLOAT16, 2, w3_rows, 64, 9 * 128, 64, 64, 128)) return e;
+  if (const char* e = tma_encode_im2col(&tm1, act1, 32, 16, 16, static_cast<uint64_t>(grid) * A1S * 2, 2, 128,
+                                        CU_TENSOR_MAP_SWIZZLE_64B))
+    return e;
+  if (const char* e = tma_encode_im2col(&tm2, act2, 64, 8, 8, static_cast<uint64_t>(grid) * A2S * GROUP, 2, 128,
+                                        CU_TENSOR_MAP_SWIZZLE_128B))
+    return e;
   if (!smem_opt_in(visual_cnn_tc_kernel, TC_SMEM)) return "visual_cnn_tc: cudaFuncSetAttribute failed";
   CnnTcDev d;
   d.frames = frames; d.pooled = reinterpret_cast<__nv_bfloat16*>(pooled);
   d.w1 = w.w1; d.b1 = w.b1; d.w2_slabs = w2_slabs; d.b2 = w.b2; d.b3 = w.b3;
+  d.act1 = act1; d.act2 = act2;
   d.M = M; d.num_groups = (M + GROUP - 1) / GROUP;
   d.trace = trace;
   d.frame_lens = frame_lens; d.N = N;
-  const int grid = d.num_groups < num_sms ? d.num_groups : num_sms;
-  launch_pdl(visual_cnn_tc_kernel, dim3(grid), dim3(TC_THREADS), TC_SMEM, s, tm, d);
+  launch_pdl(visual_cnn_tc_kernel, dim3(grid), dim3(TC_THREADS), TC_SMEM, s, tm, tm1, tm2, d);
   return cudaGetLastError() == cudaSuccess ? nullptr : "visual_cnn_tc: launch failed";
 }
 
```

After: 485,000 (median of 6 runs). No clear change (+0.7%).
